# lh3/miniwfa

Measured on AMD Instinct MI355X. Metric: aligned Gbp/s (q+t), higher is better.
Workload: dtype int16x2 packed, range-guarded (bit-exact to the reference's int32); 1 GPU; 1024 pairs/GPU x 10000 bp, 0.05 divergence, score-only mwf_wfa_exact, default penalties (BASELINE configs[2]); pairs_this_gpu=1024, pairs_total=1024, target_len=10000, bases_this_gpu=20479492, grid=512, block=512

## Files before the change

miniwfa_amd/build.py:

```python
from __future__ import annotations

import os
import subprocess
import sys

HERE = os.path.dirname(os.path.abspath(__file__))
ROOT = os.path.dirname(HERE)
CSRC = os.path.join(HERE, "csrc")
LIB = os.path.join(CSRC, "libmwf_hip.so")
SOURCES = ["mwf_band2.hip", "mwf_band2_e3.hip", "mwf_band2_e4.hip", "mwf_band2_bi.hip", "mwf_band2_bi_deep.hip", "mwf_kernels.hip", "mwf_lane.hip", "mwf_mid.hip", "mwf_sys.hip", "mwf_sys_deep.hip", "mwf_cigar_ops.hip", "mwf_engine.cpp", "mwf_memory.cpp", "mwf_plan.cpp", "mwf_chain.cpp", "mwf_async.cpp", "kalloc.cpp", "mwf_dbg.cpp"]
HEADERS = [os.path.join(CSRC, "mwf_internal.h"), os.path.join(CSRC, "mwf_device.h"), os.path.join(CSRC, "mwf_sys_pass.h"), os.path.join(CSRC, "mwf_engine.h"), os.path.join(ROOT, "include", "miniwfa.h"), os.path.join(ROOT, "include", "kalloc.h")]
SOURCE_DEPS = {"mwf_band2_e3.hip": ["mwf_band2.hip"], "mwf_band2_e4.hip": ["mwf_band2.hip"], "mwf_band2_bi.hip": ["mwf_band2.hip"], "mwf_band2_bi_deep.hip": ["mwf_band2.hip"]}


def hipcc() -> str:
    for cand in (os.environ.get("HIPCC"), "/opt/rocm/bin/hipcc", "hipcc"):
        if cand and (os.path.isabs(cand) and os.path.exists(cand) or not os.path.isabs(cand)):
            return cand
    return "hipcc"


def stale() -> bool:
    if not os.path.exists(LIB):
        return True
    t = os.path.getmtime(LIB)
    deps = [os.path.join(CSRC, s) for s in SOURCES if os.path.exists(os.path.join(CSRC, s))] + HEADERS + [os.path.abspath(__file__)]
    return any(os.path.getmtime(d) > t for d in deps)


def build(force: bool = False, verbose: bool = False) -> str:
    if not force and not stale():
        return LIB
    from concurrent.futures import ThreadPoolExecutor
    objdir = os.path.join(CSRC, "build")
    os.makedirs(objdir, exist_ok=True)
    flags = ["--offload-arch=gfx950", "-O3", "-std=c++17", "-fPIC", "-Wall", "-Wno-unused-function", "-I", os.path.join(ROOT, "include"), "-I", CSRC]
    hdr_time = max(os.path.getmtime(h) for h in HEADERS + [os.path.abspath(__file__)])
    jobs, objs = [], []
    for name in SOURCES:
        src = os.path.join(CSRC, name)
        if not os.path.exists(src):
            continue
        obj = os.path.join(objdir, name + ".o")
        objs.append(obj)
        src_time = max(os.path.getmtime(os.path.join(CSRC, d)) for d in [name, *SOURCE_DEPS.get(name, [])])
        if force or not os.path.exists(obj) or os.path.getmtime(obj) < max(src_time, hdr_time):
            jobs.append([hipcc(), *flags, "-c", src, "-o", obj])

    def run(cmd):
        if verbose:
            print(" ".join(cmd))
        return cmd, subprocess.run(cmd, capture_output=True, text=True)

    with ThreadPoolExecutor(max(1, min(6, len(jobs)))) as ex:
        for cmd, r in ex.map(run, jobs):
            if r.returncode != 0:
                sys.stderr.write(r.stdout + r.stderr)
                raise RuntimeError("hipcc failed: " + " ".join(cmd))
            if verbose and r.stderr.strip():
                sys.stderr.write(r.stderr)
    cmd, r = run([hipcc(), "--offload-arch=gfx950", "-fPIC", "-shared", *objs, "-o", LIB + ".tmp", "-lpthread"])
    if r.returncode != 0:
        sys.stderr.write(r.stdout + r.stderr)
        raise RuntimeError("hipcc failed linking libmwf_hip.so")
    os.replace(LIB + ".tmp", LIB)
    return LIB


KERNEL_FILES = {"wfa_band2_kernel": "mwf_band2.hip", "wfa_sys_kernel": "mwf_sys.hip", "wfa_sys_seg_kernel": "mwf_sys.hip", "wfa_batch_kernel": "mwf_kernels.hip",
                "wfa_lane_kernel": "mwf_lane.hip", "wfa_mid_kernel": "mwf_mid.hip"}
KERNEL_HEADERS = {"mwf_sys.hip": ["mwf_sys_pass.h", "mwf_sys_deep.hip"], "mwf_band2.hip": ["mwf_band2_e3.hip", "mwf_band2_e4.hip", "mwf_band2_bi.hip", "mwf_band2_bi_deep.hip"]}


def kernel_fingerprint(symbol: str) -> str | None:
    import hashlib
    name = symbol.split("<")[0].strip()
    f = KERNEL_FILES.get(name)
    if f is None:
        return None
    h = hashlib.sha256()
    for p in [os.path.join(CSRC, x) for x in [f, *KERNEL_HEADERS.get(f, []), "mwf_device.h", "mwf_internal.h"]]:
        try:
            h.update(open(p, "rb").read())
        except OSError:
            return None
    return h.hexdigest()[:16]


CLI = os.path.join(ROOT, "tools", "test-mwf")


def build_cli(force: bool = False) -> str:
    src = os.path.join(ROOT, "tools", "test-mwf.cpp")
    if not force and os.path.exists(CLI) and os.path.getmtime(CLI) >= max(os.path.getmtime(src), os.path.getmtime(LIB)):
        return CLI
    zl = ["-DMWF_HAVE_ZLIB", "-lz"] if os.path.exists("/usr/include/zlib.h") else []
    cmd = ["g++", "-O2", "-std=c++17", "-Wall", "-I", os.path.join(ROOT, "include"), src, "-o", CLI,
           "-L", CSRC, "-lmwf_hip", "-Wl,-rpath," + CSRC] + zl
    r = subprocess.run(cmd, capture_output=True, text=True)
    if r.returncode != 0:
        sys.stderr.write(r.stdout + r.stderr)
        raise RuntimeError("g++ failed building tools/test-mwf")
    return CLI


if __name__ == "__main__":
    print(build(force="--force" in sys.argv, verbose=True))
    print(build_cli(force="--force" in sys.argv))
```

miniwfa_amd/csrc/mwf_band2.hip:

```cpp
#include <cstddef>
#include <cstdio>
#include <cstdlib>
#include <type_traits>
#include "mwf_device.h"

namespace mwf {

using namespace dev;

namespace {

extern __shared__ __attribute__((aligned(16))) uint8_t lds2[];

constexpr int kWideT = 512, kWideK = 3;
constexpr int kWaves768 = 1;
constexpr int kSpanK = 5;
constexpr int kW4K = 5;
constexpr int kSpanT = 1024;
constexpr bool is_span(int T, int K) { return T == kSpanT && K == kSpanK; }
constexpr int kWideWaves = 4;
constexpr int kChunk = 256;
constexpr int kFoldMaxLag = 8;
constexpr int32_t kDeadPair = (int32_t)0x80008000u;

__device__ __forceinline__ int32_t from_left(int32_t v, int32_t fill) { return __builtin_amdgcn_update_dpp(fill, v, 0x138, 0xf, 0xf, false); }
__device__ __forceinline__ int32_t from_right(int32_t v, int32_t fill) { return __builtin_amdgcn_update_dpp(fill, v, 0x130, 0xf, 0xf, false); }
__device__ __forceinline__ int32_t lo16(int32_t v) { return (int32_t)(int16_t)(v & 0xffff); }
__device__ __forceinline__ int32_t hi16(int32_t v) { return v >> 16; }
__device__ __forceinline__ int32_t pack2(int32_t a, int32_t b)
{
	typedef short short2_t __attribute__((ext_vector_type(2)));
	const short2_t v = __builtin_amdgcn_cvt_pk_i16(a, b);
	return __builtin_bit_cast(int32_t, v);
}
__device__ __forceinline__ int32_t both16(int32_t v) { return (int32_t)(((uint32_t)v << 16) | ((uint32_t)v & 0xffffu)); }

__device__ __forceinline__ uint32_t seq4(int32_t off)
{
	const uint32_t *p = (const uint32_t*)(lds2 + (off & ~3));
	return __builtin_amdgcn_alignbyte(p[1], p[0], (uint32_t)off);
}

__device__ __forceinline__ int32_t lead_eq(uint32_t x)
{
	int32_t fb;
	asm("v_ffbl_b32 %0, %1" : "=v"(fb) : "v"(x));
	return (int32_t)((uint32_t)fb >> 3);
}

template <bool WANT_TB>
__device__ __forceinline__ Cell cell16(int32_t hx, int32_t o1m, int32_t g1m, int32_t o2m, int32_t g2m,
                                       int32_t o1p, int32_t g1p, int32_t o2p, int32_t g2p)
{
	if (!WANT_TB) return wf_cell<false>(hx, o1m, g1m, o2m, g2m, o1p, g1p, o2p, g2p);
	Cell c;
	c.e1 = max(o1m, g1m);
	c.e2 = max(o2m, g2m);
	c.f1 = max(o1p, g1p) + 1;
	c.f2 = max(o2p, g2p) + 1;
	const int32_t e = max(c.e1, c.e2), f = max(c.f1, c.f2), g = max(e, f), m = hx + 1;
	c.h = max(m, g);
	const uint32_t z = c.h == m ? 0u : c.h == c.e1 ? 1u : c.h == c.e2 ? 3u : c.h == c.f1 ? 2u : 4u;
	c.tb = z | ((uint32_t)(c.e1 != o1m) << 3) | ((uint32_t)(c.f1 != o1p + 1) << 4) | ((uint32_t)(c.e2 != o2m) << 5) | ((uint32_t)(c.f2 != o2p + 1) << 6);
	(void)e, (void)f, (void)g;
	return c;
}

struct Probe8 { uint32_t t0, t1, t2, q0, q1, q2; };
__device__ __forceinline__ void probe8_issue(Probe8 &p, int32_t j, int32_t aq)
{
	const uint32_t *pt = (const uint32_t*)(lds2 + (j & ~3)), *pq = (const uint32_t*)(lds2 + (aq & ~3));
	p.t0 = pt[0], p.t1 = pt[1], p.t2 = pt[2], p.q0 = pq[0], p.q1 = pq[1], p.q2 = pq[2];
}
__device__ __forceinline__ int32_t probe8_count(const Probe8 &p, int32_t j, int32_t aq)
{
	const uint32_t x0 = __builtin_amdgcn_alignbyte(p.t1, p.t0, (uint32_t)j) ^ __builtin_amdgcn_alignbyte(p.q1, p.q0, (uint32_t)aq);
	const uint32_t x1 = __builtin_amdgcn_alignbyte(p.t2, p.t1, (uint32_t)j) ^ __builtin_amdgcn_alignbyte(p.q2, p.q1, (uint32_t)aq);
	return min(min(lead_eq(x0), lead_eq(x1) + 4), 9);
}

__device__ __forceinline__ uint32_t seq16(int32_t base, int32_t j)
{
	const uint32_t *p = (const uint32_t*)(lds2 + base + ((j >> 4) << 2));
	return __builtin_amdgcn_alignbit(p[1], p[0], (uint32_t)j << 1);
}
__device__ __forceinline__ int32_t lead_eq2(uint32_t x)
{
	int32_t fb;
	asm("v_ffbl_b32 %0, %1" : "=v"(fb) : "v"(x));
	return (int32_t)((uint32_t)fb >> 1);
}
struct Probe16 { uint32_t t0, t1, q0, q1; };
__device__ __forceinline__ void probe16_issue(Probe16 &p, int32_t qbase, int32_t j, int32_t iq)
{
	const uint32_t *pt = (const uint32_t*)(lds2 + ((j >> 4) << 2)), *pq = (const uint32_t*)(lds2 + qbase + ((iq >> 4) << 2));
	p.t0 = pt[0], p.t1 = pt[1], p.q0 = pq[0], p.q1 = pq[1];
}
__device__ __forceinline__ int32_t probe16_count(const Probe16 &p, int32_t j, int32_t iq)
{
	return min(lead_eq2(__builtin_amdgcn_alignbit(p.t1, p.t0, (uint32_t)j << 1) ^ __builtin_amdgcn_alignbit(p.q1, p.q0, (uint32_t)iq << 1)), 17);
}
__device__ __forceinline__ int32_t run_wave16(int32_t qbase, int32_t j, int32_t iq, int32_t room, int32_t n0)
{
	const int32_t lane = threadIdx.x & 63;
	int32_t n = n0;
	while (n < room) {
		const int32_t off = n + 16 * lane;
		int32_t m = 0;
		if (off < room) m = min(min(lead_eq2(seq16(0, j + off) ^ seq16(qbase, iq + off)), 16), room - off);
		const unsigned long long stop = __ballot(m < 16);
		if (stop == 0) { n += 1024; continue; }
		const int32_t first = (int32_t)__builtin_ctzll(stop);
		n += 16 * first + __builtin_amdgcn_readlane(m, first);
		break;
	}
	return min(n, room);
}
template <int T>
__device__ __forceinline__ uint32_t pack2bit(const uint8_t *src, int32_t len, int32_t base)
{
	uint32_t bad = 0;
	const int32_t n_dw = (len >> 4) + 2;
	for (int32_t w = threadIdx.x; w < n_dw; w += T) {
		uint32_t out = 0;
		const int32_t b0 = w << 4;
		if (b0 + 16 <= len) {
			uint32_t q[4];
			__builtin_memcpy(q, src + b0, 16);
#pragma unroll
			for (int k = 0; k < 4; ++k) {
				const uint32_t x = q[k], code = (x >> 1) & 0x03030303u;
				const uint32_t lo1 = code & 0x01010101u, hi1 = (code >> 1) & 0x01010101u;
				const uint32_t expect = 0x41414141u + (lo1 & ~hi1) * 0x02u + (hi1 & ~lo1) * 0x13u + (hi1 & lo1) * 0x06u;
				bad |= x ^ expect;
				out |= ((code | code >> 6 | code >> 12 | code >> 18) & 0xffu) << (8 * k);
			}
		} else {
#pragma unroll 1
			for (int32_t k = 0; k < 16 && b0 + k < len; ++k) {
				const uint32_t x = src[b0 + k], code = (x >> 1) & 3u;
				bad |= x ^ ((0x47544341u >> (8 * code)) & 0xffu);
				out |= code << (2 * k);
			}
		}
		*(uint32_t*)(lds2 + base + 4 * w) = out;
	}
	return bad;
}

__device__ __forceinline__ uint32_t inm_bit(int32_t d, int32_t k, int32_t tl, int32_t ql)
{
	return (uint32_t)((uint32_t)(k + 1) < (uint32_t)(tl + 1)) & (uint32_t)((uint32_t)(d + k + 1) < (uint32_t)(ql + 1));
}

__device__ __forceinline__ unsigned long long lane_mask(int32_t base, int32_t k, int32_t a, int32_t b)
{
	int32_t lmin = a - base - k, lmax = b - base - k;
	if (lmax < 0) return 0ull;
	lmin = lmin <= 0 ? 0 : (lmin + 3) >> 2;
	lmax = min(lmax >> 2, 63);
	if (lmin > lmax) return 0ull;
	return (~0ull >> (63 - lmax)) & (~0ull << lmin);
}

__device__ __forceinline__ int32_t run_wave2(int32_t j, int32_t aq, int32_t room, int32_t n0)
{
	const int32_t lane = threadIdx.x & 63;
	int32_t n = n0;
	while (n < room) {
		const int32_t off = n + 4 * lane;
		int32_t m = 0;
		if (off < room) {
			const uint32_t x = seq4(j + off) ^ seq4(aq + off);
			m = min(min(lead_eq(x), 4), room - off);
		}
		const unsigned long long stop = __ballot(m < 4);
		if (stop == 0) { n += 256; continue; }
		const int32_t first = (int32_t)__builtin_ctzll(stop);
		n += 4 * first + __builtin_amdgcn_readlane(m, first);
		break;
	}
	return min(n, room);
}

constexpr int32_t kBiasOver = 1500, kBiasMargin = 600;
__device__ __forceinline__ int32_t wide_bias(int32_t tl) { return max(tl + kBiasOver - 32767, 0); }

template <int D, int NWK>
struct alignas(16) Band2Lds {
	Shared sh;
	int32_t edge[D][NWK + 2][4];
	int32_t dump[64 * 2 + (2 * NWK + 4) * 4];
};

typedef short s16x2 __attribute__((ext_vector_type(2)));
typedef unsigned short u16x2 __attribute__((ext_vector_type(2)));
#define MWF_BC(T, v) __builtin_bit_cast(T, v)
__device__ __forceinline__ int32_t pk_max(int32_t a, int32_t b) { return MWF_BC(int32_t, __builtin_elementwise_max(MWF_BC(s16x2, a), MWF_BC(s16x2, b))); }
__device__ __forceinline__ int32_t pk_add(int32_t a, int32_t b) { return MWF_BC(int32_t, (s16x2)(MWF_BC(s16x2, a) + MWF_BC(s16x2, b))); }
__device__ __forceinline__ int32_t pk_sub(int32_t a, int32_t b) { return MWF_BC(int32_t, (s16x2)(MWF_BC(s16x2, a) - MWF_BC(s16x2, b))); }
__device__ __forceinline__ int32_t pk_minu(int32_t a, int32_t b) { return MWF_BC(int32_t, __builtin_elementwise_min(MWF_BC(u16x2, a), MWF_BC(u16x2, b))); }
__device__ __forceinline__ int32_t pk_subsat(int32_t a, int32_t b) { return MWF_BC(int32_t, __builtin_elementwise_sub_sat(MWF_BC(u16x2, a), MWF_BC(u16x2, b))); }
__device__ __forceinline__ int32_t pk_nonzero_mask(int32_t x)
{
	int32_t m;
	asm("v_pk_min_u16 %0, %1, 1 op_sel_hi:[1,0]\n\tv_pk_sub_i16 %0, 0, %0 op_sel_hi:[0,1]" : "=&v"(m) : "v"(x));
	return m;
}
__device__ __forceinline__ int32_t pk_ne1(int32_t a, int32_t b)
{
	int32_t m;
	asm("v_xor_b32 %0, %1, %2\n\tv_pk_min_u16 %0, %0, 1 op_sel_hi:[1,0]" : "=&v"(m) : "v"(a), "v"(b));
	return m;
}
__device__ __forceinline__ int32_t pk_mad(int32_t a, int32_t b, int32_t c)
{
	int32_t m;
	asm("v_pk_mad_u16 %0, %1, %2, %3" : "=v"(m) : "v"(a), "v"(b), "v"(c));
	return m;
}
__device__ __forceinline__ int32_t bfi(int32_t mask, int32_t a, int32_t b) { return (a & mask) | (b & ~mask); }
__device__ __forceinline__ int32_t half_of(int32_t v, int hi) { return hi ? v >> 16 : (int32_t)(int16_t)(v & 0xffff); }
__device__ __forceinline__ int32_t pair_of(int32_t lo, int32_t hi) { return (int32_t)(((uint32_t)hi << 16) | ((uint32_t)lo & 0xffffu)); }

__device__ __forceinline__ int32_t left_of_A(int32_t B, int32_t fill) { return __builtin_amdgcn_alignbit(B, from_left(B, fill), 16); }
__device__ __forceinline__ int32_t right_of_B(int32_t A, int32_t fill) { return __builtin_amdgcn_alignbit(from_right(A, fill), A, 16); }

template <int T, int K, int E1, int E2, bool TB, bool S2, bool BI4, bool FOLD, typename ArgsT>
__device__ PassResult band2_pass(const ArgsT &A, const PairMem &M, Shared &sh, const int32_t edge_base, const int32_t qoff, bool trace_band)
{
	constexpr int NW = T / 64, NWK = NW * K, D = (E1 > E2 ? E1 : E2) + 1;
	constexpr bool BI = is_span(T, K) || BI4;
	constexpr int FULL = S2 ? 16 : 8;
	constexpr int kAgeOut = FOLD ? kFoldMaxLag : D;
	constexpr int kAge = (NWK + 2) * 16;
	static_assert(D >= 2 && D <= 5, "edge-table ages");
	const int32_t tl = M.tl, ql = M.ql, cmax = tl + ql + 1;
	const int32_t tid = threadIdx.x, lane = tid & 63, wave = uni(tid >> 6);
	const int32_t W = A.W, nH = A.pen.nH, lagx = A.pen.x, lag1 = A.pen.oe1, lag2 = A.pen.oe2;
	const int32_t B = BI ? wide_bias(tl) : 0;
	const int32_t ONEB = BI ? both16(1 + B) : 0x00010001;
	char *const Hb = (char*)M.H;
	const uint32_t RS = (uint32_t)W << 1;
	const int32_t min_lag = min(lagx, min(lag1, lag2));
	const bool relaxed_stores = min_lag >= 3;
	PassResult R;
	R.status = ST_OK, R.s = 0, R.info = 0, R.n_snap = 0, R.cells = 0;

	static_assert(E1 >= 1 && E1 <= 4 && (E2 == 1 || E2 == 2), "history depth");
	int32_t e1h[E1][K][2], f1h[E1][K][2], e2h[E2][K][2], f2h[E2][K][2];
#pragma unroll
	for (int k = 0; k < K; ++k)
#pragma unroll
		for (int i = 0; i < 2; ++i) {
#pragma unroll
			for (int a = 0; a < E1; ++a) e1h[a][k][i] = f1h[a][k][i] = kDeadPair;
#pragma unroll
			for (int a = 0; a < E2; ++a) e2h[a][k][i] = f2h[a][k][i] = kDeadPair;
		}
	const int32_t RA = pair_of(4 * lane, 4 * lane + 2);
	const uint32_t lane8 = ((uint32_t)lane << 3) + 8u;
	const int32_t nd = lane == 0 ? -4 : 8;
	const int32_t T0 = both16(cmax), TLp = both16(tl), TL1 = both16(tl + 1);
	const int32_t ebase = edge_base + wave * 16, dump_base = edge_base + D * kAge + NW * 16;
	const int32_t dump_lane = dump_base + lane * 8;
	int32_t epos[D];
#pragma unroll
	for (int a = 0; a < D; ++a) epos[a] = a * kAge;

	{
		const int32_t reach = nH + 1 + 8, g_a = max(tl + 1 - reach, 0) >> 8, n_g = ((tl + 1 + reach) >> 8) - g_a + 1, per_row = n_g * 64;
		for (int32_t q = tid; q < nH * per_row; q += T) {
			const int32_t row = q / per_row, rem = q - row * per_row;
			*(int2*)(Hb + (size_t)((uint32_t)row * RS + (uint32_t)(g_a * 512 + rem * 8 + 8))) = make_int2(kDeadPair, kDeadPair);
		}
	}
	for (int32_t j = tid; j < D * (NWK + 2) * 4; j += T) *(int32_t*)(lds2 + edge_base + 4 * j) = kDeadPair;
	if (tid == 0) {
		for (int32_t j = 0; j < nH; ++j) sh.rng_lo[j] = 1, sh.rng_hi[j] = 0;
		for (int32_t j = 0; j < 12; ++j) (&sh.flags[0][0])[j] = 0;
		sh.rng_lo[0] = sh.rng_hi[0] = tl + 1;
		sh.word[3] = -1;
	}
	__syncthreads();
	if (tid < 64) {
		const int32_t k0 = (S2 ? run_wave16(qoff, 0, 0, min(tl, ql), 0) : run_wave2(0, qoff, min(tl, ql), 0)) - 1;
		if (tid == 0) {
			const int32_t c = tl + 1, e = c & 3;
			*(int16_t*)(Hb + 8 + (size_t)(uint32_t)(((c & ~3) + ((e & 1) << 1) + (e >> 1)) << 1)) = (int16_t)(k0 - B);
			sh.word[1] = k0;
		}
	}
	__syncthreads();
	{
		const int32_t k0 = uni(sh.word[1]);
		if (k0 == tl - 1 && k0 == ql - 1) return R;
	}

	int32_t s = 0, wf_lo = tl + 1, wf_hi = tl + 1;
	int32_t curH = 0, par = 0;
	const uint32_t ring_bytes = (uint32_t)nH * RS;
	uint32_t bn = (uint32_t)(1 % nH) * RS, bx = (uint32_t)((nH - lagx + 1) % nH) * RS, b1 = (uint32_t)((nH - lag1 + 1) % nH) * RS, b2 = (uint32_t)((nH - lag2 + 1) % nH) * RS;
	struct Rows { int2 HX, O1, O2; int32_t N1, N2; } pre;
	pre.HX = pre.O1 = pre.O2 = make_int2(0, 0), pre.N1 = pre.N2 = 0;
	auto load_rows = [&](Rows &r, const char *rx, const char *r1, const char *r2, uint32_t off) {
		const uint32_t noff = off + (uint32_t)nd;
		r.HX = *(const int2*)(rx + off), r.O2 = *(const int2*)(r2 + off);
		r.N2 = *(const int32_t*)(r2 + noff);
		if (!FOLD) r.O1 = *(const int2*)(r1 + off), r.N1 = *(const int32_t*)(r1 + noff);
	};
	int64_t cells = 0, tb_used = 0;
	int32_t est_window = 0;
	const int64_t iter_limit = A.max_iter > 0 ? A.max_iter : INT64_MAX;
	const int32_t s_limit = A.max_s > 0 ? A.max_s : INT32_MAX;
	const int64_t rows_slot = TB ? A.rows_slot : 0, tb_slot_bytes = TB ? A.tb_slot_bytes : 0;

	int32_t gl = (wf_lo > 1 ? wf_lo - 1 : 1) >> 8, gk[K];
	auto remap = [&](int32_t g_lo) {
		const int32_t base = g_lo - g_lo % NWK;
#pragma unroll
		for (int k = 0; k < K; ++k) {
			int32_t g = base + wave + NW * k;
			if (g < g_lo) g += NWK;
			gk[k] = g;
		}
	};
	remap(gl);
	int32_t idle[K];
#pragma unroll
	for (int k = 0; k < K; ++k) idle[k] = kAgeOut;
	int32_t up_wait = 0, up_min = 0;
	int32_t ekey = 0;
	constexpr bool kEpoch = !is_span(T, K) && T != 64;
	uint32_t est = 0;
	static_assert(kEpoch || ((NW & (NW - 1)) == 0 && !(T == 512 && K == 4)), "the full header of the gated geometries is written for a power-of-two wave count and no three-slot note");
	static_assert(K <= 6, "slot classes of the window epoch: four bits per slot below bit 24");

	auto step = [&]() __attribute__((always_inline)) -> bool {
		constexpr int P1 = E1 - 1, P2 = E2 - 1;
#ifdef MWF_B2_TIMING
		const uint64_t tm0 = __builtin_readcyclecounter();
#endif
		const int32_t lo = wf_lo > 1 ? wf_lo - 1 : 1;
		const int32_t hi = wf_hi < cmax ? wf_hi + 1 : cmax;
		const int32_t lo_p = lo, hi_p = hi;
		const int32_t s_new = s + 1;
		const int32_t newH = curH + 1 == nH ? 0 : curH + 1;
		const int32_t npar = par + 1 == 3 ? 0 : par + 1;
		const int32_t origin = lo & ~3;
		const int32_t row_bytes = (hi | 3) - origin + 1;
		if (TB) {
			if (s_new - 1 >= rows_slot) { R.status = ST_ROWS_OVERFLOW; return true; }
			if (tb_used + row_bytes > tb_slot_bytes) { R.status = ST_TB_OVERFLOW; return true; }
		}
		const int32_t gl_next = (lo > 1 ? lo - 1 : 1) >> 8;
		const int32_t ga = lo >> 8, gb = hi >> 8;
		const int32_t key = gl_next | gb << 15 | 1 << 29 | (ga - gl_next) << 30;
		const bool fast = kEpoch && key == ekey;
		uint32_t st = est;
		bool act[K];
		if (!kEpoch) {
			if (gb - min(ga, gl + 1) + 3 > NWK - 1)
				if (((hi < cmax ? hi + 1 : cmax) >> 8) - min(gl_next, gl) + 1 > NWK - 1) { R.status = ST_BAND_OVERFLOW; return true; }
			if (BI && cmax - lo > 65535) { R.status = ST_BAND_OVERFLOW; return true; }
		} else if (!fast) {
			bool hold = true;
			if (gb - min(ga, gl + 1) + 3 > NWK - 1) {
				if (((hi < cmax ? hi + 1 : cmax) >> 8) - min(gl_next, gl) + 1 > NWK - 1) { R.status = ST_BAND_OVERFLOW; return true; }
				hold = false;
			}
			if (T == 512 && K == 4 && R.n_snap == 0 && gb - ga + 3 > 23) {
				if (((hi < cmax ? hi + 1 : cmax) >> 8) - gl_next + 1 > 23) R.n_snap = 1;
				hold = false;
			}
			if (BI) {
				if (cmax - lo > 65535) { R.status = ST_BAND_OVERFLOW; return true; }
				if (cmax - (ga << 8) > 65535) hold = false;
			}
			const int32_t gspan = gb - ga;
			int n_busy = 0;
			st = 0;
#pragma unroll
			for (int k = 0; k < K; ++k) {
				if ((uint32_t)(gk[k] - ga) <= (uint32_t)gspan) {
					idle[k] = 0;
					st |= (1u | (gk[k] == ga ? 2u : 0u) | (gk[k] == gb ? 4u : 0u)) << (4 * k);
					if (k < 2 || k == K - 1) ++n_busy;
				} else if (idle[k] < kAgeOut) {
					++idle[k];
					st |= 9u << (4 * k);
					hold = false;
				}
			}
			if ((NW & (NW - 1)) == 0) {
				const int32_t pos = (wave - ga) & (NW - 1);
				const int32_t left = gspan + 1 - pos + ((pos == 0 || ((gb - wave) & (NW - 1)) == 0) ? NW : 0);
				if (left > 2 * NW) __builtin_amdgcn_s_setprio(3);
				else if (left > NW) __builtin_amdgcn_s_setprio(2);
				else if (left > 0) __builtin_amdgcn_s_setprio(1);
				else __builtin_amdgcn_s_setprio(0);
			} else {
				if (n_busy >= 3) __builtin_amdgcn_s_setprio(3);
				else if (n_busy == 2) __builtin_amdgcn_s_setprio(2);
				else if (n_busy == 1) __builtin_amdgcn_s_setprio(1);
				else __builtin_amdgcn_s_setprio(0);
			}
			if (ga >= 1 && wave == (ga - 1) % NW) st |= 1u << 24;
			if (wave == (gb + 1) % NW) st |= 1u << 25;
			est = st, ekey = kEpoch && hold ? ~key : -1;
		}
		const char *const rowx = Hb + bx, *const row1 = Hb + b1, *const row2 = Hb + b2;
		char *const rown = Hb + bn;
		const bool track_good = (((256 - (s_new & 255)) & 255) < nH);
		const int32_t rE1 = ebase + epos[E1 - 1], rE2 = ebase + epos[E2 - 1];
		const int32_t wE = lane == 63 ? ebase + epos[D - 1] : dump_lane, wF = lane == 0 ? ebase + epos[D - 1] : dump_lane;
		auto put_edge = [&](int k, int32_t e1b, int32_t e2b, int32_t f1a, int32_t f2a) {
			*(int2*)(lds2 + wE + (k * NW + 1) * 16) = make_int2(e1b, e2b);
			*(int2*)(lds2 + wF + (k * NW + 1) * 16 + 8) = make_int2(f1a, f2a);
			if (k == K - 1 && wave == NW - 1) *(int2*)(lds2 + wE - (NW - 1) * 16) = make_int2(e1b, e2b);
			if (k == 0 && wave == 0) *(int2*)(lds2 + wF + (NWK + 1) * 16 + 8) = make_int2(f1a, f2a);
		};
		const bool forecast = NWK < 24 ? (s_new == 64 || s_new == 256 || s_new == 1024) : NWK >= 64 ? (s_new == 1024 || s_new == 4096) : false;
		int32_t far = kDeadPair;
		const int32_t cfin = ql + 1;

		if (wave == 0) {
			sh.rng_lo[newH] = lo, sh.rng_hi[newH] = hi;
			sh.flags[npar + 1 == 3 ? 0 : npar + 1][0] = 0;
			if (TB) M.row_off[s_new - 1] = tb_used, M.row_lo[s_new - 1] = origin;
#ifndef MWF_B2_TIMING
			if (trace_band && s_new - 1 < fresh(A).dbg_cap) M.dbg[2 * (s_new - 1)] = lo, M.dbg[2 * (s_new - 1) + 1] = hi;
#endif
		}

		if (!kEpoch) {
#pragma unroll
			for (int k = 0; k < K; ++k) act[k] = (uint32_t)(gk[k] - ga) <= (uint32_t)(gb - ga);
			const int32_t pos = (wave - ga) & (NW - 1);
			const int32_t left = gb - ga + 1 - pos + ((pos == 0 || ((gb - wave) & (NW - 1)) == 0) ? NW : 0);
			if (left > 2 * NW) __builtin_amdgcn_s_setprio(3);
			else if (left > NW) __builtin_amdgcn_s_setprio(2);
			else if (left > 0) __builtin_amdgcn_s_setprio(1);
			else __builtin_amdgcn_s_setprio(0);
		}
#ifdef MWF_B2_TIMING
		int n_act = 0;
#pragma unroll
		for (int k = 0; k < K; ++k) n_act += (kEpoch ? (st >> (4 * k) & 9u) == 1u : act[k]) ? 1 : 0;
#endif

#ifdef MWF_B2_TIMING
		const uint64_t tm1 = __builtin_readcyclecounter();
#endif
		int n_stores = 0;
		if (kEpoch ? (st & (1u << 24)) != 0 : (ga >= 1 && wave == (ga - 1) % NW)) *(int2*)(rown + ((uint32_t)((ga - 1) << 9) + lane8)) = make_int2(kDeadPair, kDeadPair);
		if (kEpoch ? (st & (1u << 25)) != 0 : wave == (gb + 1) % NW) *(int2*)(rown + ((uint32_t)((gb + 1) << 9) + lane8)) = make_int2(kDeadPair, kDeadPair);
#if MWF_B2_TIMING == 2
		bool chunk_timed = false;
		uint32_t ct[4] = {0, 0, 0, 0};
#endif
#pragma unroll
		for (int k = 0; k < K; ++k) {
			const uint32_t cls = st >> (4 * k);
			if (kEpoch) {
				if (!(cls & 1u)) continue;
			} else if (!act[k]) {
				if (idle[k] >= kAgeOut) continue;
				++idle[k];
			} else idle[k] = 0;
			const bool edgy = (cls & 0xeu) != 0;
			int32_t lo = uni(lo_p), hi = uni(hi_p);
			asm volatile("" : "+s"(lo), "+s"(hi));
			const int32_t g = gk[k], cb = g * kChunk, c0 = cb + 4 * lane;
#if MWF_B2_TIMING == 2
			uint64_t tc0 = 0, tc1 = 0, tc2 = 0, tc3 = 0, tc4 = 0;
			const bool timed = !chunk_timed;
			if (timed) asm volatile("s_memtime %0\n\ts_waitcnt lgkmcnt(0)" : "=s"(tc0) :: "memory");
#endif
			const uint32_t off = (uint32_t)(cb << 1) + lane8;
			load_rows(pre, rowx, row1, row2, off);
			const int2 HX = pre.HX, O1 = pre.O1, O2 = pre.O2;
			const int32_t N1 = pre.N1, N2 = pre.N2;
			const int32_t xE1 = *(const int32_t*)(lds2 + rE1 + k * NW * 16), xE2 = *(const int32_t*)(lds2 + rE2 + k * NW * 16 + 4);
			const int32_t xF1 = *(const int32_t*)(lds2 + rE1 + (k * NW + 2) * 16 + 8), xF2 = *(const int32_t*)(lds2 + rE2 + (k * NW + 2) * 16 + 12);
			const bool inside = (kEpoch && !edgy) || (cb >= lo && cb + kChunk - 1 <= hi);

			const int32_t E1a = e1h[P1][k][0], E1b = e1h[P1][k][1], F1a = f1h[P1][k][0], F1b = f1h[P1][k][1];
			const int32_t E2a = e2h[P2][k][0], E2b = e2h[P2][k][1], F2a = f2h[P2][k][0], F2b = f2h[P2][k][1];
			const int32_t o1mA = FOLD ? 0 : left_of_A(O1.y, N1), o2mA = left_of_A(O2.y, N2), g1mA = left_of_A(E1b, xE1), g2mA = left_of_A(E2b, xE2);
			const int32_t o1pB = FOLD ? 0 : right_of_B(O1.x, N1), o2pB = right_of_B(O2.x, N2), g1pB = right_of_B(F1a, xF1), g2pB = right_of_B(F2a, xF2);
			const int32_t ONE = 0x00010001;
			int32_t ne1A = FOLD ? g1mA : pk_max(o1mA, g1mA), ne2A = pk_max(o2mA, g2mA);
			int32_t ne1B = FOLD ? E1a : pk_max(O1.x, E1a), ne2B = pk_max(O2.x, E2a);
			const int32_t pf1A = FOLD ? F1b : pk_max(O1.y, F1b), pf2A = pk_max(O2.y, F2b);
			const int32_t pf1B = FOLD ? g1pB : pk_max(o1pB, g1pB), pf2B = pk_max(o2pB, g2pB);
			int32_t nf1A = pk_add(pf1A, ONE), nf2A = pk_add(pf2A, ONE), nf1B = pk_add(pf1B, ONE), nf2B = pk_add(pf2B, ONE);
			const int32_t mA = pk_add(HX.x, ONE), mB = pk_add(HX.y, ONE);
			int32_t hA = pk_max(pk_max(mA, pk_max(ne1A, ne2A)), pk_max(nf1A, nf2A));
			int32_t hB = pk_max(pk_max(mB, pk_max(ne1B, ne2B)), pk_max(nf1B, nf2B));
#if MWF_B2_TIMING == 2
			if (timed) asm volatile("s_memtime %0\n\ts_waitcnt lgkmcnt(0)" : "=s"(tc1) : "v"(hA), "v"(hB) : "memory");
#endif
			uint32_t tbw = 0;
			if (TB) {
				const int32_t TWO = 0x00020002, NEG1 = (int32_t)0xffffffffu, EIGHT = 0x00080008, C16 = 0x00100010, C32 = 0x00200020, C64 = 0x00400040;
				int32_t zA = pk_mad(pk_ne1(hA, nf1A), TWO, NEG1), zB = pk_mad(pk_ne1(hB, nf1B), TWO, NEG1);
				zA = pk_mad(pk_ne1(hA, ne2A), zA, TWO), zB = pk_mad(pk_ne1(hB, ne2B), zB, TWO);
				zA = pk_mad(pk_ne1(hA, ne1A), zA, ONE), zB = pk_mad(pk_ne1(hB, ne1B), zB, ONE);
				zA = pk_mad(pk_ne1(hA, mA), zA, 0), zB = pk_mad(pk_ne1(hB, mB), zB, 0);
				if (!FOLD) {
					zA = pk_mad(pk_ne1(ne1A, o1mA), EIGHT, zA), zB = pk_mad(pk_ne1(ne1B, O1.x), EIGHT, zB);
					zA = pk_mad(pk_ne1(pf1A, O1.y), C16, zA), zB = pk_mad(pk_ne1(pf1B, o1pB), C16, zB);
				}
				zA = pk_mad(pk_ne1(ne2A, o2mA), C32, zA), zB = pk_mad(pk_ne1(ne2B, O2.x), C32, zB);
				zA = pk_mad(pk_ne1(pf2A, O2.y), C64, zA), zB = pk_mad(pk_ne1(pf2B, o2pB), C64, zB);
				tbw = (uint32_t)zA | ((uint32_t)zB << 8);
			}
			const int32_t cbp = both16(cb);
			const int32_t xA = pk_sub(pk_sub(T0, cbp), RA);
			const int32_t rjA = pk_minu(xA, TLp), rjB = pk_minu(pk_sub(xA, ONE), TLp);
			const int32_t dA = pk_sub(pk_add(RA, cbp), TL1), dB = pk_add(dA, ONE);
			const bool on_lo = kEpoch ? (cls & 2u) != 0 : g == ga, on_hi = kEpoch ? (cls & 4u) != 0 : g == gb;
			const bool special = is_span(T, K) || (BI4 && !TB) || (kEpoch ? edgy : !inside || on_lo || on_hi) || track_good;
			int32_t outA = 0, outB = 0;
			uint32_t bits = 0, gbits = 0;
			if (special) {
			if (!inside) {
				const int32_t lo_r = both16(min(max(lo - cb, 0), 256)), hi_r1 = both16(min(max(hi - cb + 1, 0), 256));
				const int32_t RB = pk_add(RA, 0x00010001), RB1 = pk_add(RA, 0x00020002);
				outA = pk_nonzero_mask(pk_subsat(lo_r, RA) | pk_subsat(RB, hi_r1));
				outB = pk_nonzero_mask(pk_subsat(lo_r, RB) | pk_subsat(RB1, hi_r1));
				hA = bfi(outA, kDeadPair, hA), hB = bfi(outB, kDeadPair, hB);
				ne1A = bfi(outA, kDeadPair, ne1A), ne1B = bfi(outB, kDeadPair, ne1B);
				ne2A = bfi(outA, kDeadPair, ne2A), ne2B = bfi(outB, kDeadPair, ne2B);
				nf1A = bfi(outA, kDeadPair, nf1A), nf1B = bfi(outB, kDeadPair, nf1B);
				nf2A = bfi(outA, kDeadPair, nf2A), nf2B = bfi(outB, kDeadPair, nf2B);
			}
			if (on_lo || on_hi) {
				if (on_lo) {
					const int32_t rel = lo - cb;
					const int32_t v = half_of(__builtin_amdgcn_readlane((rel & 1) ? hB : hA, rel >> 2), (rel >> 1) & 1);
					bits |= v >= -1 - B ? 1u : 0u;
				}
				if (on_hi) {
					const int32_t rel = hi - cb;
					const int32_t v = half_of(__builtin_amdgcn_readlane((rel & 1) ? hB : hA, rel >> 2), (rel >> 1) & 1);
					bits |= v >= -1 - B ? 2u : 0u;
				}
			}
			if (track_good) {
				auto bad = [&](int32_t v, int32_t rj) { return pk_subsat(pk_add(v, ONEB), rj); };
				const int32_t bA = pk_minu(pk_minu(bad(hA, rjA), pk_minu(bad(ne1A, rjA), bad(nf1A, rjA))), pk_minu(bad(ne2A, rjA), bad(nf2A, rjA))) | outA;
				const int32_t bB = pk_minu(pk_minu(bad(hB, rjB), pk_minu(bad(ne1B, rjB), bad(nf1B, rjB))), pk_minu(bad(ne2B, rjB), bad(nf2B, rjB))) | outB;
				gbits = (uint32_t)((bA & 0xffff) == 0) | (uint32_t)((bB & 0xffff) == 0) << 1 | (uint32_t)(((uint32_t)bA >> 16) == 0) << 2 | (uint32_t)(((uint32_t)bB >> 16) == 0) << 3;
				if (BI && (s_new & 255) == 0) {
					const int32_t width = both16(kBiasMargin), from = both16(-1 - B - kBiasMargin), top = both16(32768 - kBiasMargin);
					auto stray = [&](int32_t v, int32_t lo_end) { return pk_subsat(width, pk_sub(v, lo_end)); };
					const int32_t any = stray(hA, from) | stray(hB, from) | stray(ne1A, from) | stray(ne1B, from) | stray(ne2A, from) | stray(ne2B, from) |
					                    stray(nf1A, from) | stray(nf1B, from) | stray(nf2A, from) | stray(nf2B, from) | stray(hA, top) | stray(hB, top);
					if (__ballot(any != 0)) bits |= 0x80u;
				}
			}
			}
			if (FOLD) {
				ne1A = pk_max(ne1A, HX.x), ne1B = pk_max(ne1B, HX.y), nf1A = pk_max(nf1A, HX.x), nf1B = pk_max(nf1B, HX.y);
				if (TB) {
					const int32_t EIGHT = 0x00080008, C16 = 0x00100010;
					const int32_t fA = pk_mad(pk_ne1(ne1A, HX.x), EIGHT, pk_mad(pk_ne1(nf1A, HX.x), C16, 0));
					const int32_t fB = pk_mad(pk_ne1(ne1B, HX.y), EIGHT, pk_mad(pk_ne1(nf1B, HX.y), C16, 0));
					tbw |= (uint32_t)fA | ((uint32_t)fB << 8);
				}
			}
			e1h[P1][k][0] = ne1A, e1h[P1][k][1] = ne1B, f1h[P1][k][0] = nf1A, f1h[P1][k][1] = nf1B;
			e2h[P2][k][0] = ne2A, e2h[P2][k][1] = ne2B, f2h[P2][k][0] = nf2A, f2h[P2][k][1] = nf2B;
#pragma unroll
			for (int i = 0; i < 2; ++i) {
#pragma unroll
				for (int a = E1 - 1; a > 0; --a) {
					asm volatile("v_swap_b32 %0, %1" : "+v"(e1h[a - 1][k][i]), "+v"(e1h[a][k][i]));
					asm volatile("v_swap_b32 %0, %1" : "+v"(f1h[a - 1][k][i]), "+v"(f1h[a][k][i]));
				}
#pragma unroll
				for (int a = E2 - 1; a > 0; --a) {
					asm volatile("v_swap_b32 %0, %1" : "+v"(e2h[a - 1][k][i]), "+v"(e2h[a][k][i]));
					asm volatile("v_swap_b32 %0, %1" : "+v"(f2h[a - 1][k][i]), "+v"(f2h[a][k][i]));
				}
			}
			put_edge(k, ne1B, ne2B, nf1A, nf2A);

#if MWF_B2_TIMING == 2
			if (timed) asm volatile("s_memtime %0\n\ts_waitcnt lgkmcnt(0)" : "=s"(tc2) : "v"(hA), "v"(hB), "v"(rjA), "v"(dA) : "memory");
#endif
			const int32_t jA = pk_minu(pk_add(hA, ONEB), rjA), jB = pk_minu(pk_add(hB, ONEB), rjB);
			const int32_t iqA = pk_add(jA, dA), iqB = pk_add(jB, dB);
			int32_t cnt[4];
			if (S2) {
				uint64_t tw[4], qw[4];
#pragma unroll
				for (int u = 0; u < 4; ++u) {
					const uint32_t J = (uint32_t)((u & 1) ? jB : jA), Q = (uint32_t)((u & 1) ? iqB : iqA);
					const uint32_t ta = (u & 2) ? (J >> 18) & 0x3ffcu : (J >> 2) & 0x3ffcu;
					const uint32_t qa = ((u & 2) ? (Q >> 20) : ((Q >> 4) & 0xfffu)) * 4u + (uint32_t)qoff;
					asm volatile("ds_read2_b32 %0, %1 offset1:1" : "=v"(tw[u]) : "v"(ta));
					asm volatile("ds_read2_b32 %0, %1 offset1:1" : "=v"(qw[u]) : "v"(qa));
				}
				asm volatile("s_waitcnt lgkmcnt(0)" : "+v"(tw[0]), "+v"(tw[1]), "+v"(tw[2]), "+v"(tw[3]), "+v"(qw[0]), "+v"(qw[1]), "+v"(qw[2]), "+v"(qw[3]));
#pragma unroll
				for (int u = 0; u < 4; ++u) {
					const uint32_t J = (uint32_t)((u & 1) ? jB : jA), Q = (uint32_t)((u & 1) ? iqB : iqA);
					const uint32_t tsh = (u & 2) ? (BI ? (J >> 15) & 30u : J >> 15) : J << 1, qsh = (u & 2) ? (Q >> 15) & 30u : Q << 1;
					cnt[u] = lead_eq2(__builtin_amdgcn_alignbit((uint32_t)(tw[u] >> 32), (uint32_t)tw[u], tsh) ^ __builtin_amdgcn_alignbit((uint32_t)(qw[u] >> 32), (uint32_t)qw[u], qsh));
				}
			} else {
				constexpr int PF = (K >= 3 && T >= 512) ? 1 : 2;
#pragma unroll
				for (int h2 = 0; h2 < 4 / PF; ++h2) {
					Probe8 pr[PF];
					int32_t jj[PF], aq[PF];
#pragma unroll
					for (int v = 0; v < PF; ++v) {
						const int u = PF * h2 + v;
						jj[v] = (int32_t)((uint32_t)((u & 1) ? jB : jA) >> ((u & 2) ? 16 : 0) & 0xffffu);
						aq[v] = (int32_t)((uint32_t)((u & 1) ? iqB : iqA) >> ((u & 2) ? 16 : 0) & 0xffffu) + qoff;
						probe8_issue(pr[v], jj[v], aq[v]);
					}
#pragma unroll
					for (int v = 0; v < PF; ++v) cnt[PF * h2 + v] = probe8_count(pr[v], jj[v], aq[v]);
				}
			}
			typedef unsigned short us2_t __attribute__((ext_vector_type(2)));
			const int32_t cA = MWF_BC(int32_t, (us2_t)__builtin_amdgcn_cvt_pk_u16((uint32_t)cnt[0], (uint32_t)cnt[2]));
			const int32_t cB = MWF_BC(int32_t, (us2_t)__builtin_amdgcn_cvt_pk_u16((uint32_t)cnt[1], (uint32_t)cnt[3]));
#if MWF_B2_TIMING == 2
			if (timed) asm volatile("s_memtime %0\n\ts_waitcnt lgkmcnt(0)" : "=s"(tc3) : "v"(cA), "v"(cB) : "memory");
#endif
			const int32_t FULLp = both16(FULL);
			const int32_t m9A = pk_minu(cA, pk_sub(rjA, jA)), m9B = pk_minu(cB, pk_sub(rjB, jB));
			int32_t nmA = pk_minu(m9A, FULLp), nmB = pk_minu(m9B, FULLp);
			const int32_t pendp = pk_subsat(m9A, FULLp) | pk_subsat(m9B, FULLp);
			if (__ballot(pendp != 0)) {
				int32_t hv[4] = {half_of(hA, 0) + B, half_of(hB, 0) + B, half_of(hA, 1) + B, half_of(hB, 1) + B};
				int32_t nmat[4] = {(int32_t)((uint32_t)nmA & 0xffffu), (int32_t)((uint32_t)nmB & 0xffffu), (int32_t)((uint32_t)nmA >> 16), (int32_t)((uint32_t)nmB >> 16)};
				const uint32_t pend = (uint32_t)(((uint32_t)m9A & 0xffffu) > (uint32_t)FULL) | (uint32_t)(((uint32_t)m9B & 0xffffu) > (uint32_t)FULL) << 1 |
				                      (uint32_t)(((uint32_t)m9A >> 16) > (uint32_t)FULL) << 2 | (uint32_t)(((uint32_t)m9B >> 16) > (uint32_t)FULL) << 3;
				uint32_t open = 0;
#pragma unroll
				for (int i = 0; i < 4; ++i) {
					if (__ballot((pend >> i) & 1u) == 0) continue;
					if ((pend >> i) & 1u) {
						int32_t n = FULL;
						const int32_t j = hv[i] + 1, q = c0 + i - 1 - tl + j, rm = min(tl - j, ql - q), aqq = qoff + q;
						for (int trip = 0; n < rm; ++trip) {
							if (trip == 4) { open |= 1u << i; break; }
							if (S2) {
								const int32_t m = min(lead_eq2(seq16(0, j + n) ^ seq16(qoff, q + n)), 16);
								n += m;
								if (m < 16) break;
							} else {
								const uint32_t xa = seq4(j + n) ^ seq4(aqq + n), xb = seq4(j + n + 4) ^ seq4(aqq + n + 4);
								if (xa | xb) { n += xa ? min(lead_eq(xa), 4) : 4 + min(lead_eq(xb), 4); break; }
								n += 8;
							}
						}
						nmat[i] = min(n, rm);
					}
				}
				for (unsigned long long owners = __ballot(open != 0); owners; owners &= owners - 1) {
					const int32_t src = (int32_t)__builtin_ctzll(owners);
					const int32_t c0s = cb + 4 * src;
					const uint32_t ob = (uint32_t)__builtin_amdgcn_readlane((int32_t)open, src);
#pragma unroll
					for (int i = 0; i < 4; ++i) {
						if (!((ob >> i) & 1u)) continue;
						const int32_t hh = __builtin_amdgcn_readlane(hv[i], src);
						const int32_t j = hh + 1, q = c0s + i - 1 - tl + j, rm = min(tl - j, ql - q);
						const int32_t n = S2 ? run_wave16(qoff, j, q, rm, 80) : run_wave2(j, qoff + q, rm, 40);
						nmat[i] = lane == src ? n : nmat[i];
					}
				}
				nmA = pair_of(nmat[0], nmat[2]), nmB = pair_of(nmat[1], nmat[3]);
			}
			const int32_t hxA = pk_add(hA, nmA), hxB = pk_add(hB, nmB);
			if (forecast) far = pk_max(far, pk_max(hxA, hxB));
			unsigned long long fm = 0;
			int32_t done_info = 0;
			if ((uint32_t)(cfin - cb) < (uint32_t)kChunk && cfin >= lo && cfin <= hi) {
				const int32_t rel = cfin - cb, hi_half = (rel >> 1) & 1;
				const int32_t hv = half_of((rel & 1) ? hxB : hxA, hi_half) + B, nm = (int32_t)((uint32_t)((rel & 1) ? nmB : nmA) >> (hi_half ? 16 : 0) & 0xffffu);
				const uint32_t f = (uint32_t)(lane == (rel >> 2)) & (uint32_t)(hv == tl - 1) & inm_bit(ql - tl, hv - nm, tl, ql);
				done_info = (f && nm == 0) ? (int32_t)((tbw >> (8 * (rel & 3))) & 7u) : 0;
				fm = __ballot(f != 0);
			}
			*(int2*)(rown + off) = make_int2(hxA, hxB);
			++n_stores;
#if MWF_B2_TIMING == 2
			if (timed) {
				asm volatile("s_memtime %0\n\ts_waitcnt lgkmcnt(0)" : "=s"(tc4) : "v"(hxA), "v"(hxB) : "memory");
				chunk_timed = true;
				ct[0] = (uint32_t)min(tc1 - tc0, (uint64_t)4095), ct[1] = (uint32_t)min(tc2 - tc1, (uint64_t)4095);
				ct[2] = (uint32_t)min(tc3 - tc2, (uint64_t)4095), ct[3] = (uint32_t)min(tc4 - tc3, (uint64_t)4095);
			}
#endif
			if (TB && c0 >= origin && c0 <= hi) *(uint32_t*)(M.tb + tb_used - origin + c0) = tbw;
			if (track_good) {
				unsigned long long *gword = M.good + (int64_t)newH * fresh(A).GW + g * 4;
#pragma unroll
				for (int i = 0; i < 4; ++i) {
					const unsigned long long m = __ballot((gbits >> i) & 1u);
					if (lane == 0) gword[i] = m;
				}
			}
			if (fm) bits |= 4u | (uint32_t)__builtin_amdgcn_readlane(done_info, (int32_t)__builtin_ctzll(fm)) << 4;
			if (bits && lane == 0) atomicOr((unsigned int*)&sh.flags[npar][0], bits);
		}

		if (forecast) {
			const int32_t m = wave_max(max(lo16(far), hi16(far))) + B;
			if (lane == 0 && m >= 0) atomicMax(&sh.word[3], m);
		}
#ifdef MWF_B2_TIMING
		const uint64_t tm2 = __builtin_readcyclecounter();
#endif
		bn = bn + RS == ring_bytes ? 0u : bn + RS, bx = bx + RS == ring_bytes ? 0u : bx + RS;
		b1 = b1 + RS == ring_bytes ? 0u : b1 + RS, b2 = b2 + RS == ring_bytes ? 0u : b2 + RS;
		const bool young_store = relaxed_stores && n_stores > 0 && !TB && !track_good;
		if (young_store) asm volatile("s_waitcnt vmcnt(1) lgkmcnt(0)" ::: "memory");
		else asm volatile("s_waitcnt vmcnt(0) lgkmcnt(0)" ::: "memory");
#ifdef MWF_B2_TIMING
		const uint64_t tm3 = __builtin_readcyclecounter();
#endif
		__builtin_amdgcn_s_barrier();
		asm volatile("" ::: "memory");

		const uint32_t fl = (uint32_t)uni(sh.flags[npar][0]);
#ifdef MWF_B2_TIMING
		if (trace_band && tid == (fresh(A).max_iter < 0 ? (int32_t)-fresh(A).max_iter : 0) && s_new - 1 < fresh(A).dbg_cap) {
			const uint64_t tm4 = __builtin_readcyclecounter();
#if MWF_B2_TIMING == 2
			M.dbg[2 * (s_new - 1)] = (int32_t)(ct[0] | ct[1] << 12 | (uint32_t)n_act << 28);
			M.dbg[2 * (s_new - 1) + 1] = (int32_t)(ct[2] | ct[3] << 12);
			(void)tm4;
#else
			M.dbg[2 * (s_new - 1)] = (int32_t)(min((uint32_t)(tm1 - tm0), 65535u) | min((uint32_t)(tm2 - tm1), 65535u) << 16);
			M.dbg[2 * (s_new - 1) + 1] = (int32_t)(min((uint32_t)(tm3 - tm2), 4095u) | min((uint32_t)(tm4 - tm3), 65535u) << 12 | (uint32_t)n_act << 28);
#endif
		}
#endif
		if (fl & 1u) wf_lo = lo;
		if (fl & 2u) wf_hi = hi;
		const int32_t done = (int32_t)((fl >> 2) & 1u), payload = (int32_t)((fl >> 4) & 7u);
		if (BI && (fl & 0x80u)) { R.status = ST_BAND_OVERFLOW; return true; }
		s = s_new, curH = newH, par = npar;
		{
			const int32_t oldest = epos[D - 1];
#pragma unroll
			for (int a = D - 1; a > 0; --a) epos[a] = epos[a - 1];
			epos[0] = oldest;
		}
		if (!kEpoch || ekey < 0) {
			if (gl_next < gl) gl = gl_next, remap(gl), up_wait = 0, ekey = 0;
			else if (gl_next > gl) {
				up_min = up_wait == 0 ? gl_next : min(up_min, gl_next);
				if (++up_wait > kAgeOut) gl = up_min, remap(gl), up_wait = 0;
				ekey = 0;
			} else up_wait = 0, ekey = ~ekey;
		}
		if (TB) tb_used += row_bytes;
		if ((s & 0xff) == 0) {
			if (tid == 0) sh.red[0] = 0x7fffffff, sh.red[1] = -1;
			__syncthreads();
			const int32_t gfirst = wf_lo >> 8, n_words = ((wf_hi >> 8) - gfirst + 1) * 4, GWc = fresh(A).GW;
			for (int32_t q = tid; q < n_words; q += T) {
				const int32_t gg = gfirst + (q >> 2), kq = q & 3, base = gg * kChunk;
				unsigned long long m = 0;
				for (int32_t j = 0; j < nH; ++j)
					if (sh.rng_lo[j] <= sh.rng_hi[j] && sh.rng_lo[j] <= base + kChunk - 1 && sh.rng_hi[j] >= base) m |= M.good[(int64_t)j * GWc + gg * 4 + kq];
				m &= lane_mask(base, kq, wf_lo, wf_hi);
				if (m) {
					atomicMin(&sh.red[0], base + 4 * (int32_t)__builtin_ctzll(m) + kq);
					atomicMax(&sh.red[1], base + 4 * (63 - (int32_t)__builtin_clzll(m)) + kq);
				}
			}
			__syncthreads();
			const int32_t glo = uni(sh.red[0]), ghi = uni(sh.red[1]);
			if (ghi < 0) { R.status = ST_INTERNAL; return true; }
			wf_lo = glo, wf_hi = ghi;
		}
		cells += hi - lo + 1;
		if (cells > iter_limit || s > s_limit) {
			R.status = ST_STOPPED;
			return true;
		}
		if (done) {
			R.info = payload;
			return true;
		}
		if (forecast) {
			est_window = window_forecast(s, uni(sh.word[3]), tl, ql, (NWK - 1) * kChunk - 64, NWK >= 24 && NWK < 64);
			if (est_window) { R.status = ST_BAND_OVERFLOW; return true; }
		}
		return false;
	};
	for (;;)
		if (step()) break;
	asm volatile("s_waitcnt vmcnt(0)" ::: "memory");
	R.s = s, R.cells = est_window ? -(int64_t)est_window : cells;
	return R;
}

constexpr int band2_waves(int T, int K, bool TB)
{
	return is_span(T, K) ? (T == 1024 ? 4 : 3) : T == 1024 ? 4 : T == kWideT ? kWideWaves : T <= 512 ? ((TB && T < 512) ? 3 : 4) : kWaves768;
}
template <int T, int K, int E1, int E2, bool TB, bool S2, bool BI4 = false, bool FOLD = false>
__global__ __launch_bounds__(T, band2_waves(T, K, TB)) void wfa_band2_kernel(const BatchArgs)
{
	constexpr int NWK = (T / 64) * K, D = (E1 > E2 ? E1 : E2) + 1;
	KArgs &A0 = kernel_args();
	if ((uint32_t)(uintptr_t)lds2 != 0u) __builtin_trap();
	typedef Band2Lds<D, NWK> LdsT;
	const int32_t lds_seq = A0.band_lds_seq;
	LdsT *const L = (LdsT*)(lds2 + lds_seq);
	Shared &sh = L->sh;
	const int32_t edge_base = lds_seq + (int32_t)offsetof(LdsT, edge);
	CigLocal cig_loc;
	cig_loc.base = 0, cig_loc.left = 0;
	for (int32_t round = 0;; ++round) {
		KArgs &A = fresh(A0);
		if (threadIdx.x == 0) sh.item = A.queue ? (int32_t)atomicAdd(A.queue, 1) : (round == 0 ? (int32_t)blockIdx.x : A.n_pairs), sh.word[2] = 0;
		__syncthreads();
		const int32_t item = uni(sh.item);
		__syncthreads();
		if (item >= A.n_pairs) break;
		const int32_t pair = A.order ? A.order[item] : item;
		PairMem M;
		pair_mem(A, (int32_t)blockIdx.x, pair, M);
		const int32_t qoff = S2 ? ((M.tl >> 4) + 2) * 4 : ((M.tl + 3) & ~3) + 8;
		PassResult R;
		R.status = ST_OK, R.s = 0, R.info = 0, R.n_snap = 0, R.cells = 0;
		if (S2) {
			uint32_t bad = pack2bit<T>(M.ts, M.tl, 0);
			bad |= pack2bit<T>(M.qs, M.ql, qoff);
			if (bad) sh.word[2] = 1;
			__syncthreads();
			if (uni(sh.word[2])) R.status = ST_ALPHABET;
		} else {
			for (int32_t j = threadIdx.x; j < M.tl; j += T) lds2[j] = M.ts[j];
			for (int32_t j = threadIdx.x; j < M.ql; j += T) lds2[qoff + j] = M.qs[j];
			__syncthreads();
		}
		const bool trace = A.dbg && pair == A.debug_pair;
		if (R.status == ST_OK) R = band2_pass<T, K, E1, E2, TB, S2, BI4, FOLD>(A, M, sh, edge_base, qoff, trace);
		if (T == 512 && K == 4 && R.n_snap && threadIdx.x == 0 && fresh(A0).report_wide) atomicOr((unsigned int*)(fresh(A0).cig_head + 1), 1u);
		R.n_snap = 0;
		if (S2) M.t2 = lds2, M.q2 = lds2 + qoff;
		if (TB && FOLD) M.tb_fwd = 1;
		finish_pair(fresh(A0), M, (int32_t)blockIdx.x, pair, R, R.status, 0, T <= 256 ? &cig_loc : nullptr);
	}
}

template <int T, int K, int E1, int E2>
constexpr int lds_tail() { return (int)sizeof(Band2Lds<(E1 > E2 ? E1 : E2) + 1, (T / 64) * K>); }

template <int T, int K, int E1, int E2, bool TB, bool S2, bool BI4 = false, bool FOLD = false>
void launch_variant(const BatchArgs &a, int grid, int lds, hipStream_t st)
{
	if constexpr (!FOLD && T >= 512 && S2 && E1 == 2) {
		if (a.band_fold && a.pen.oe1 - a.pen.x == E1 && a.pen.oe1 < kFoldMaxLag) return launch_variant<T, K, E1, E2, TB, S2, BI4, true>(a, grid, lds, st);
	}
	if (lds > 48 * 1024) {
		(void)hipFuncSetAttribute(reinterpret_cast<const void*>(&wfa_band2_kernel<T, K, E1, E2, TB, S2, BI4, FOLD>), hipFuncAttributeMaxDynamicSharedMemorySize, lds);
		(void)hipGetLastError();
	}
	if (getenv("MWF_DEBUG"))
		fprintf(stderr, "[libmwf_hip] band2 launch: T %d K %d E1 %d E2 %d TB %d S2 %d BI4 %d FOLD %d, %d pairs, grid %d\n", T, K, E1, E2, (int)TB, (int)S2, (int)BI4, (int)FOLD, (int)a.n_pairs, grid);
	hipLaunchKernelGGL((wfa_band2_kernel<T, K, E1, E2, TB, S2, BI4, FOLD>), dim3(grid), dim3(T), lds, st, a);
}

template <int T, int K, int E1, int E2, bool BI4 = false>
int launch_one(const BatchArgs &a0, int grid, int lds_seq, bool seq2, hipStream_t st)
{
	BatchArgs a = a0;
	a.band_lds_seq = lds_seq;
	const int lds = lds_seq + lds_tail<T, K, E1, E2>();
	if constexpr (is_span(T, K) || (T == 512 && K >= 4)) {
		if (!seq2) return -1;
		if (a.want_cigar) launch_variant<T, K, E1, E2, true, true, BI4>(a, grid, lds, st);
		else launch_variant<T, K, E1, E2, false, true, BI4>(a, grid, lds, st);
	} else if constexpr (T == 768) {
		if (seq2) return -1;
		if (a.want_cigar) launch_variant<T, K, E1, E2, true, false>(a, grid, lds, st);
		else launch_variant<T, K, E1, E2, false, false>(a, grid, lds, st);
	} else {
		if (!seq2) return -1;
		if (a.want_cigar) launch_variant<T, K, E1, E2, true, true>(a, grid, lds, st);
		else launch_variant<T, K, E1, E2, false, true>(a, grid, lds, st);
	}
	return hipGetLastError() == hipSuccess ? 0 : -2;
}

template <int T, int K, int E1, int E2, bool BI4 = false>
int occ_one(int lds_seq, bool seq2, bool tb)
{
	const int lds = lds_seq + lds_tail<T, K, E1, E2>();
	int n = 0;
	hipError_t e;
	if constexpr (is_span(T, K) || (T == 512 && K >= 4)) {
		if (!seq2) return 0;
		e = tb ? hipOccupancyMaxActiveBlocksPerMultiprocessor(&n, wfa_band2_kernel<T, K, E1, E2, true, true, BI4>, T, lds)
		       : hipOccupancyMaxActiveBlocksPerMultiprocessor(&n, wfa_band2_kernel<T, K, E1, E2, false, true, BI4>, T, lds);
	} else if constexpr (T == 768) {
		if (seq2) return 0;
		e = tb ? hipOccupancyMaxActiveBlocksPerMultiprocessor(&n, wfa_band2_kernel<T, K, E1, E2, true, false>, T, lds)
		       : hipOccupancyMaxActiveBlocksPerMultiprocessor(&n, wfa_band2_kernel<T, K, E1, E2, false, false>, T, lds);
	} else {
		if (!seq2) return 0;
		e = tb ? hipOccupancyMaxActiveBlocksPerMultiprocessor(&n, wfa_band2_kernel<T, K, E1, E2, true, true>, T, lds)
		       : hipOccupancyMaxActiveBlocksPerMultiprocessor(&n, wfa_band2_kernel<T, K, E1, E2, false, true>, T, lds);
	}
	return e == hipSuccess ? n : 0;
}

}

#define MWF_BAND2_CAT_(a, b) a##b
#define MWF_BAND2_CAT(a, b) MWF_BAND2_CAT_(a, b)
int launch_band2_e3(const BatchArgs &a, int grid, const BandGeom &g, void *stream);
int launch_band2_e4(const BatchArgs &a, int grid, const BandGeom &g, void *stream);
int band2_occupancy_e3(const Penalty &p, const BandGeom &g, bool cigar);
int band2_occupancy_e4(const Penalty &p, const BandGeom &g, bool cigar);
int launch_band2_bi1(const BatchArgs &a, int grid, const BandGeom &g, void *stream);
int launch_band2_bi2(const BatchArgs &a, int grid, const BandGeom &g, void *stream);
int band2_occupancy_bi1(const Penalty &p, const BandGeom &g, bool cigar);
int band2_occupancy_bi2(const Penalty &p, const BandGeom &g, bool cigar);

#if !defined(MWF_BAND2_DEEP) && !defined(MWF_BAND2_BIASED)
bool band2_supported(const Penalty &p)
{
	const bool deep = (p.e1 == 3 && (p.e2 == 1 || p.e2 == 2)) || (p.e1 == 4 && p.e2 == 1);
	return ((p.e1 == 2 && p.e2 == 1) || (p.e1 == 2 && p.e2 == 2) || (p.e1 == 1 && p.e2 == 1) || deep) && p.nH <= kMaxRing;
}
#endif

#if defined(MWF_BAND_DEV) || defined(MWF_BAND2_BIASED)
#define MWF_BAND2_REST(FN, ...)
#else
#define MWF_BAND2_REST(FN, ...)                                                     \
	if (g.block == 256) MWF_BAND2_PEN(FN, 256, 3, __VA_ARGS__)                      \
	if (g.block == 128) MWF_BAND2_PEN(FN, 128, 3, __VA_ARGS__)                      \
	if (g.block == 64) MWF_BAND2_PEN(FN, 64, 3, __VA_ARGS__)
#endif
#if defined(MWF_BAND2_BIASED)
#define MWF_BAND2_PEN(FN, T, K, ...) {}
#elif defined(MWF_BAND2_DEEP) && MWF_BAND2_DEEP == 3
#define MWF_BAND2_PEN(FN, T, K, ...)                                                \
	{                                                                               \
		if (a_e1 == 3 && a_e2 == 1) return FN<T, K, 3, 1>(__VA_ARGS__);             \
		if (a_e1 == 3 && a_e2 == 2) return FN<T, K, 3, 2>(__VA_ARGS__);             \
	}
#elif defined(MWF_BAND2_DEEP)
#define MWF_BAND2_PEN(FN, T, K, ...)                                                \
	{                                                                               \
		if (a_e1 == MWF_BAND2_DEEP && a_e2 == 1) return FN<T, K, MWF_BAND2_DEEP, 1>(__VA_ARGS__); \
	}
#elif defined(MWF_BAND_DEV)
#define MWF_BAND2_PEN(FN, T, K, ...) { if (a_e1 == 2 && a_e2 == 1) return FN<T, K, 2, 1>(__VA_ARGS__); }
#else
#define MWF_BAND2_PEN(FN, T, K, ...)                                                \
	{                                                                               \
		if (a_e1 == 2 && a_e2 == 1) return FN<T, K, 2, 1>(__VA_ARGS__);             \
		if (a_e1 == 2 && a_e2 == 2) return FN<T, K, 2, 2>(__VA_ARGS__);             \
		if (a_e1 == 1 && a_e2 == 1) return FN<T, K, 1, 1>(__VA_ARGS__);             \
	}
#endif
#if defined(MWF_BAND2_BIASED) && MWF_BAND2_BIASED == 1
#define MWF_BAND2_PEN4(FN, K, ...)                                                  \
	{                                                                               \
		if (a_e1 == 2 && a_e2 == 2) return FN<512, K, 2, 2, true>(__VA_ARGS__);     \
		if (a_e1 == 1 && a_e2 == 1) return FN<512, K, 1, 1, true>(__VA_ARGS__);     \
	}
#elif defined(MWF_BAND2_BIASED)
#define MWF_BAND2_PEN4(FN, K, ...)                                                  \
	{                                                                               \
		if (a_e1 == 3 && a_e2 == 1) return FN<512, K, 3, 1, true>(__VA_ARGS__);     \
		if (a_e1 == 3 && a_e2 == 2) return FN<512, K, 3, 2, true>(__VA_ARGS__);     \
		if (a_e1 == 4 && a_e2 == 1) return FN<512, K, 4, 1, true>(__VA_ARGS__);     \
	}
#endif
#if defined(MWF_BAND2_BIASED)
#define MWF_BAND2_PEN4B(FN, ...) MWF_BAND2_PEN4(FN, kW4K, __VA_ARGS__)
#define MWF_BAND2_PEN4C(FN, ...) MWF_BAND2_PEN4(FN, kW4K + 1, __VA_ARGS__)
#elif defined(MWF_BAND2_DEEP)
#define MWF_BAND2_PEN4B(FN, ...) {}
#define MWF_BAND2_PEN4C(FN, ...) {}
#else
#define MWF_BAND2_PEN4B(FN, ...)                                                    \
	{                                                                               \
		if (a_e1 == 2 && a_e2 == 1) return FN<512, kW4K, 2, 1, true>(__VA_ARGS__);     \
	}
#define MWF_BAND2_PEN4C(FN, ...)                                                    \
	{                                                                               \
		if (a_e1 == 2 && a_e2 == 1) return FN<512, kW4K + 1, 2, 1, true>(__VA_ARGS__); \
	}
#endif
#define MWF_BAND2_DISPATCH(FN, ...)                                                 \
	do {                                                                            \
		if (g.block == 512 && g.span > 8 * kW4K * 256 && g.packed == 2) MWF_BAND2_PEN4C(FN, __VA_ARGS__)  \
		if (g.block == 512 && g.span > 512 / 64 * 3 * 256 && g.packed == 2) MWF_BAND2_PEN4B(FN, __VA_ARGS__)  \
		if (g.block == 512 && g.span > 512 / 64 * 3 * 256) MWF_BAND2_PEN(FN, 512, 4, __VA_ARGS__)  \
		if (g.block == 512) MWF_BAND2_PEN(FN, kWideT, kWideK, __VA_ARGS__) \
		if (g.block == 768) MWF_BAND2_PEN(FN, 768, 2, __VA_ARGS__)                  \
		if (g.block == 1024) MWF_BAND2_PEN(FN, kSpanT, kSpanK, __VA_ARGS__) \
		MWF_BAND2_REST(FN, __VA_ARGS__)                                             \
	} while (0)

#if defined(MWF_BAND2_BIASED)
int MWF_BAND2_CAT(launch_band2_bi, MWF_BAND2_BIASED)(const BatchArgs &a, int grid, const BandGeom &g, void *stream)
{
	const int a_e1 = a.pen.e1, a_e2 = a.pen.e2;
	if (g.packed != 2) return -1;
	MWF_BAND2_DISPATCH(launch_one, a, grid, g.lds_bytes, g.seq2 != 0, (hipStream_t)stream);
	return -1;
}

int MWF_BAND2_CAT(band2_occupancy_bi, MWF_BAND2_BIASED)(const Penalty &p, const BandGeom &g, bool cigar)
{
	const int a_e1 = p.e1, a_e2 = p.e2;
	if (g.packed != 2) return 0;
	MWF_BAND2_DISPATCH(occ_one, g.lds_bytes, g.seq2 != 0, cigar);
	return 0;
}
#elif defined(MWF_BAND2_DEEP)
int MWF_BAND2_CAT(launch_band2_e, MWF_BAND2_DEEP)(const BatchArgs &a, int grid, const BandGeom &g, void *stream)
{
	const int a_e1 = a.pen.e1, a_e2 = a.pen.e2;
	if (g.packed == 2) return -1;
	MWF_BAND2_DISPATCH(launch_one, a, grid, g.lds_bytes, g.seq2 != 0, (hipStream_t)stream);
	return -1;
}

int MWF_BAND2_CAT(band2_occupancy_e, MWF_BAND2_DEEP)(const Penalty &p, const BandGeom &g, bool cigar)
{
	const int a_e1 = p.e1, a_e2 = p.e2;
	if (g.packed == 2) return 0;
	MWF_BAND2_DISPATCH(occ_one, g.lds_bytes, g.seq2 != 0, cigar);
	return 0;
}
#else
int launch_band2(const BatchArgs &a, int grid, const BandGeom &g, void *stream)
{
	const int a_e1 = a.pen.e1, a_e2 = a.pen.e2;
	if (g.packed == 2 && !(a_e1 == 2 && a_e2 == 1)) return a_e1 <= 2 ? launch_band2_bi1(a, grid, g, stream) : launch_band2_bi2(a, grid, g, stream);
	if (a_e1 == 3) return launch_band2_e3(a, grid, g, stream);
	if (a_e1 == 4) return launch_band2_e4(a, grid, g, stream);
	MWF_BAND2_DISPATCH(launch_one, a, grid, g.lds_bytes, g.seq2 != 0, (hipStream_t)stream);
	return -1;
}

int band2_span_chunks() { return kSpanT / 64 * kSpanK; }
int band2_biased512_chunks() { return 8 * kW4K; }
bool band2_biased512_supported(const Penalty &p)
{
	return (p.e1 == 2 && (p.e2 == 1 || p.e2 == 2)) || (p.e1 == 1 && p.e2 == 1) || (p.e1 == 3 && (p.e2 == 1 || p.e2 == 2)) || (p.e1 == 4 && p.e2 == 1);
}

int band2_kernel_occupancy(const Penalty &p, const BandGeom &g, bool cigar)
{
	const int a_e1 = p.e1, a_e2 = p.e2;
	if (g.packed == 2 && !(a_e1 == 2 && a_e2 == 1)) return a_e1 <= 2 ? band2_occupancy_bi1(p, g, cigar) : band2_occupancy_bi2(p, g, cigar);
	if (a_e1 == 3) return band2_occupancy_e3(p, g, cigar);
	if (a_e1 == 4) return band2_occupancy_e4(p, g, cigar);
	MWF_BAND2_DISPATCH(occ_one, g.lds_bytes, g.seq2 != 0, cigar);
	return 0;
}
#endif

}
```

miniwfa_amd/csrc/mwf_engine.cpp:

```cpp
#include "mwf_engine.h"

extern "C" {


int mwf_gpu_device_count(void)
{
	int n = 0;
	if (hipGetDeviceCount(&n) != hipSuccess) { (void)hipGetLastError(); return 0; }
	return n;
}

mwf_gpu_t *mwf_gpu_create(int device, void *stream)
{
	int n = mwf_gpu_device_count();
	if (device < 0 || device >= n) return nullptr;
	if (hipSetDevice(device) != hipSuccess) return nullptr;
	mwf_gpu_t *g = new mwf_gpu_t();
	g->device = device;
	hipDeviceProp_t prop;
	if (hipGetDeviceProperties(&prop, device) != hipSuccess) { delete g; return nullptr; }
	g->n_cu = prop.multiProcessorCount;
	g->total_mem = prop.totalGlobalMem;
	if (stream) g->stream = (hipStream_t)stream;
	else {
		if (hipStreamCreateWithFlags(&g->stream, hipStreamNonBlocking) != hipSuccess) { delete g; return nullptr; }
		g->own_stream = true;
	}
	(void)hipEventCreate(&g->ev0);
	(void)hipEventCreate(&g->ev1);
	if (ensure(g, g->queue, kQueueInts * 4) || hipMemsetAsync(g->queue.p, 0, kQueueInts * 4, g->stream) != hipSuccess) {
		mwf_gpu_destroy(g);
		return nullptr;
	}
	return g;
}

static void trim(mwf_gpu_t *g)
{
	(void)hipStreamSynchronize(g->stream);
	for (DevBuf *b : {&g->ring, &g->sring, &g->good, &g->tb, &g->row_off, &g->row_lo, &g->cig_scratch, &g->snap, &g->snap_meta, &g->seg, &g->dbg,
	                  &g->coop_edge, &g->coop_misc, &g->sys_box, &g->sys_prog, &g->sys_log, &g->sys_ep, &g->sys_park, &g->sys_ring, &g->sys_sring, &g->sys_good, &g->retry_ids,
	                  &g->spare_block, &g->spare_cig})
		release(g, *b);
	g->dev_bytes_peak = g->dev_bytes;
}

void mwf_gpu_destroy(mwf_gpu_t *g)
{
	if (!g) return;
	(void)hipSetDevice(g->device);
	trim(g);
	release(g, g->queue);
	if (g->pin) (void)hipHostFree(g->pin);
	if (g->res_pin) (void)hipHostFree(g->res_pin);
	for (hipEvent_t e : {g->ev0, g->ev1, g->pin_ev[0], g->pin_ev[1]})
		if (e) (void)hipEventDestroy(e);
	if (g->own_stream) (void)hipStreamDestroy(g->stream);
	delete g;
}

const char *mwf_gpu_last_error(const mwf_gpu_t *g) { return g ? g->err.c_str() : "no engine (no gfx950 device could be opened)"; }

int mwf_gpu_set(mwf_gpu_t *g, const char *name, int64_t value)
{
	if (!g || !name) return -1;
	if (!strcmp(name, "tb_budget_mb")) g->tb_budget_mb = value;
	else if (!strcmp(name, "lowmem_budget_mb")) g->lowmem_budget_mb = std::max<int64_t>(0, value);
	else if (!strcmp(name, "coop_min_len")) g->coop_min_len = value;
	else if (!strcmp(name, "seq2bit")) g->seq2bit = (int)value;
	else if (!strcmp(name, "ring16")) g->ring16 = (int)value;
	else if (!strcmp(name, "band_span") && value >= 0 && value <= 2) g->band_span = (int)value;
	else if (!strcmp(name, "wide_slots") && (value == 0 || value == 3 || value == 4)) g->wide_slots = (int)value;
	else if (!strcmp(name, "lane_max_len")) g->lane_max_len = (int)std::max<int64_t>(0, std::min<int64_t>(value, 8000));
	else if (!strcmp(name, "mid_max_pairs")) g->mid_max_pairs = (int)std::max<int64_t>(-1, std::min<int64_t>(value, 1 << 20));
	else if (!strcmp(name, "host_results")) g->res_pin_on = value != 0;
	else if (!strcmp(name, "div_aware")) g->div_aware = value != 0;
	else if (!strcmp(name, "dev_retry")) g->dev_retry = value != 0;
	else if (!strcmp(name, "band_fold")) g->band_fold = value != 0;
	else if (!strcmp(name, "trim")) { (void)hipSetDevice(g->device); trim(g); }
	else return -1;
	++g->tun_gen;
	return 0;
}

int mwf_gpu_test_hook(mwf_gpu_t *g, const char *name, int64_t value)
{
	if (!g || !name) return -1;
	if (!strcmp(name, "block")) {
		if (value != 0 && value != 64 && value != 128 && value != 256 && value != 512 && value != 768 && value != 1024) return -1;
		g->block = (int)value;
	} else if (!strcmp(name, "force_kind")) g->force_kind = (int)value;
	else if (!strcmp(name, "band_pack")) g->band_pack = (int)value;
	else if (!strcmp(name, "lane_chunks") && value >= 0 && value <= 4) g->lane_chunks = (int)value;
	else if (!strcmp(name, "mid_block") && (value == 0 || value == 256 || value == 512 || value == 1024)) g->mid_block = (int)value;
	else if (!strcmp(name, "lds_e2")) g->lds_e2 = value != 0;
	else if (!strcmp(name, "scalar_generic")) g->scalar_generic = value != 0;
	else if (!strcmp(name, "coop_spin_limit")) g->coop_spin_limit = std::max<int64_t>(0, std::min<int64_t>(value, 0x7fffffff));
	else if (!strcmp(name, "coop_tb_cap_mb")) g->coop_tb_cap = std::max<int64_t>(1, value) << 20;
	else if (!strcmp(name, "coop_grid")) g->coop_grid_cap = (int)std::max<int64_t>(0, value);
	else if (!strcmp(name, "sys_p") && sys_p_supported((int)value)) g->sys_p = (int)value;
	else if (!strcmp(name, "sys_c") && (value == 0 || sys_c_supported((int)value))) g->sys_c = (int)value;
	else if (!strcmp(name, "work_order") && value >= 0 && value <= 3) g->work_order = (int)value;
	else if (!strcmp(name, "timeline")) g->timeline = (int64_t*)(intptr_t)value;
	else return -1;
	++g->tun_gen;
	return 0;
}

void mwf_gpu_get_stats(const mwf_gpu_t *g, mwf_gpu_stats_t *st)
{
	if (!g || !st) return;
	mwf_gpu_t *m = const_cast<mwf_gpu_t*>(g);
	if (m->ev_pending) {
		(void)hipSetDevice(m->device);
		float ms = 0;
		if (hipEventSynchronize(m->ev1) == hipSuccess && hipEventElapsedTime(&ms, m->ev0, m->ev1) == hipSuccess) m->stats.kernel_ms = ms;
		m->ev_pending = false;
	}
	m->stats.dev_bytes = m->dev_bytes, m->stats.dev_bytes_peak = m->dev_bytes_peak;
	*st = m->stats;
}


mwf_gpu_batch_t *mwf_gpu_batch_upload(mwf_gpu_t *g, int32_t n, const char *seqs, int64_t seq_bytes,
                                      const int64_t *t_off, const int32_t *tl, const int64_t *q_off, const int32_t *ql)
{
	if (!g || n < 0 || seq_bytes < 0) return nullptr;
	return batch_from_host(g, n, tl, nullptr, ql, nullptr, seqs, seq_bytes, t_off, q_off);
}

mwf_gpu_batch_t *mwf_gpu_batch_wrap(mwf_gpu_t *g, int32_t n, const void *d_seqs, int64_t seq_bytes,
                                    const int64_t *d_t_off, const int32_t *d_tl, const int64_t *d_q_off, const int32_t *d_ql,
                                    const int32_t *h_tl, const int32_t *h_ql)
{
	if (!g || n < 0) return nullptr;
	(void)hipSetDevice(g->device);
	BlockLayout L;
	mwf_gpu_batch_t *b = batch_common(g, n, h_tl, h_ql, 0, false, L);
	if (!b) return nullptr;
	b->d_seqs = (const uint8_t*)d_seqs, b->seq_bytes = seq_bytes;
	b->d_t_off = d_t_off, b->d_q_off = d_q_off, b->d_tl = d_tl, b->d_ql = d_ql;
	if (upload_segments(g, (char*)b->block.p, std::vector<Seg>{Seg{b->h_order.data(), (size_t)n * 4}})) {
		mwf_gpu_batch_free(b);
		return nullptr;
	}
	if (g->div_aware) b->div_est = estimate_divergence_device(g, b);
	return b;
}

void mwf_gpu_batch_free(mwf_gpu_batch_t *b)
{
	if (!b) return;
	mwf_gpu_t *g = b->g;
	(void)hipSetDevice(g->device);
	if (b->busy) (void)hipStreamSynchronize(g->stream);
	if (g->res_pin_owner == b) g->res_pin_owner = nullptr;
	give_block(g, g->spare_block, b->block);
	give_block(g, g->spare_cig, b->cig);
	for (DevBuf *d : {&b->ops_summary, &b->ops_map[0], &b->ops_map[1], &b->ops_map_off[0], &b->ops_map_off[1]}) release(g, *d);
	delete b;
}

}


extern "C" {

int mwf_gpu_batch_results(mwf_gpu_t *g, mwf_gpu_batch_t *b, int32_t *s, int64_t *n_iter, int32_t *n_cigar)
{
	if (!g || !b) return -1;
	(void)hipSetDevice(g->device);
	if (int rc = finalize(g, b)) return rc;
	const size_t n = (size_t)b->n;
	if (s && n) memcpy(s, b->h_s.data(), n * 4);
	if (n_iter && n) memcpy(n_iter, b->h_iter.data(), n * 8);
	if (n_cigar && n) memcpy(n_cigar, b->h_ncig.data(), n * 4);
	return 0;
}

const int32_t *mwf_gpu_batch_dev_scores(const mwf_gpu_batch_t *b) { return b ? b->d_s : nullptr; }
const int64_t *mwf_gpu_batch_dev_iters(const mwf_gpu_batch_t *b) { return b ? b->d_iter : nullptr; }
const int32_t *mwf_gpu_batch_dev_status(const mwf_gpu_batch_t *b) { return b ? b->d_status : nullptr; }

int32_t mwf_gpu_batch_cigar(mwf_gpu_t *g, mwf_gpu_batch_t *b, int32_t i, uint32_t *dst, int32_t cap)
{
	if (!g || !b || i < 0 || i >= b->n) return -1;
	(void)hipSetDevice(g->device);
	if (int rc = finalize(g, b)) return rc;
	const int32_t nc = b->h_ncig[i];
	if (nc > cap) return -5;
	if (nc <= 0) return nc;
	if (b->h_cig_valid) memcpy(dst, b->h_cig.data() + b->h_cigoff[i], (size_t)nc * 4);
	else HIP_TRY(g, hipMemcpy(dst, b->d_cig_pool + b->h_cigoff[i], (size_t)nc * 4, hipMemcpyDeviceToHost));
	return nc;
}

int mwf_gpu_batch_fetch_cigars(mwf_gpu_t *g, mwf_gpu_batch_t *b)
{
	if (!g || !b) return -1;
	(void)hipSetDevice(g->device);
	return fetch_cigars(g, b);
}


static int own_cigars(mwf_gpu_t *g, mwf_gpu_batch_t *b, const char *who)
{
	if (int rc = finalize(g, b)) return rc;
	if (!(b->opt.flag & MWF_F_CIGAR)) { g->err = std::string(who) + ": the batch's last align was score-only (no CIGARs to work on; align with MWF_F_CIGAR)"; return -2; }
	return 0;
}

static int ops_block(mwf_gpu_batch_t *b)
{
	if (b->ops_max_len < 0) {
		b->ops_max_len = 0;
		for (int32_t i = 0; i < b->n; ++i) b->ops_max_len = std::max<int64_t>(b->ops_max_len, (int64_t)b->h_tl[i] + b->h_ql[i]);
	}
	return cigar_ops_block(b->ops_max_len);
}

static CigarOpsArgs ops_args(const mwf_gpu_batch_t *b)
{
	CigarOpsArgs a{};
	a.seqs = b->d_seqs, a.t_off = b->d_t_off, a.q_off = b->d_q_off, a.tl = b->d_tl, a.ql = b->d_ql, a.n_pairs = b->n;
	a.words = b->d_cig_pool, a.word_off = b->d_cigoff, a.n_words = b->d_ncig, a.status = b->d_status;
	return a;
}

int mwf_gpu_batch_dev_cigars(mwf_gpu_t *g, mwf_gpu_batch_t *b, const uint32_t **pool, const int64_t **word_off, const int32_t **n_words, int64_t *pool_words)
{
	if (!g || !b) return -1;
	(void)hipSetDevice(g->device);
	if (int rc = own_cigars(g, b, "mwf_gpu_batch_dev_cigars")) return rc;
	if (pool) *pool = b->d_cig_pool;
	if (word_off) *word_off = b->d_cigoff;
	if (n_words) *n_words = b->d_ncig;
	if (pool_words) *pool_words = b->n > 0 ? b->cig_used : 0;
	return 0;
}

int mwf_gpu_batch_summarize(mwf_gpu_t *g, mwf_gpu_batch_t *b, const mwf_opt_t *opt, const uint32_t *d_words, const int64_t *d_word_off, const int32_t *d_n_words)
{
	if (!g || !b) return -1;
	(void)hipSetDevice(g->device);
	const bool own = !d_words && !d_word_off && !d_n_words;
	if (!own && (!d_words || !d_word_off || !d_n_words)) { g->err = "mwf_gpu_batch_summarize: foreign CIGARs need all three device arrays (words, offsets, counts)"; return -2; }
	if (own) { if (int rc = own_cigars(g, b, "mwf_gpu_batch_summarize")) return rc; }
	else if (b->busy) HIP_TRY(g, hipStreamSynchronize(g->stream));
	if (!opt && !b->aligned) { g->err = "mwf_gpu_batch_summarize: opt == NULL needs an earlier align of the batch"; return -2; }
	const mwf_opt_t &o = opt ? *opt : b->opt;
	b->summary_valid = false;
	if (b->n == 0) { b->summary_valid = true; return 0; }
	if (ensure(g, b->ops_summary, (size_t)b->n * sizeof(mwf_aln_summary_t))) return -1;
	CigarOpsArgs a = ops_args(b);
	if (!own) a.words = d_words, a.word_off = d_word_off, a.n_words = d_n_words, a.status = nullptr;
	a.x = o.x, a.o1 = o.o1, a.e1 = o.e1, a.o2 = o.o2, a.e2 = o.e2;
	a.mode = 0, a.summary = (int32_t*)b->ops_summary.p;
	if (launch_cigar_ops(a, ops_block(b), g->stream)) { g->err = "kernel launch failed (CIGAR summary)"; return -1; }
	b->summary_valid = true;
	return 0;
}

const mwf_aln_summary_t *mwf_gpu_batch_dev_summary(const mwf_gpu_batch_t *b)
{
	return b && b->summary_valid ? (const mwf_aln_summary_t*)b->ops_summary.p : nullptr;
}

int mwf_gpu_batch_summary(mwf_gpu_t *g, mwf_gpu_batch_t *b, mwf_aln_summary_t *host_out)
{
	if (!g || !b || !host_out) return -1;
	(void)hipSetDevice(g->device);
	if (!b->summary_valid) { g->err = "mwf_gpu_batch_summary: no summary (call mwf_gpu_batch_summarize after the align)"; return -2; }
	return download(g, host_out, b->ops_summary.p, (size_t)b->n * sizeof(mwf_aln_summary_t));
}

int mwf_gpu_batch_map(mwf_gpu_t *g, mwf_gpu_batch_t *b, int32_t which)
{
	if (!g || !b || which < 0 || which > 1) return -1;
	(void)hipSetDevice(g->device);
	if (int rc = own_cigars(g, b, "mwf_gpu_batch_map")) return rc;
	b->map_valid[which] = false;
	std::vector<int64_t> &off = b->h_map_off[which];
	if (off.empty()) {
		off.assign((size_t)b->n + 1, 0);
		for (int32_t i = 0; i < b->n; ++i) off[i + 1] = off[i] + (which == 0 ? b->h_ql[i] : b->h_tl[i]);
	}
	if (b->n == 0) { b->map_valid[which] = true; return 0; }
	if (ensure(g, b->ops_map[which], std::max<size_t>((size_t)off[b->n] * 4, 256))) return -1;
	if (!b->map_off_uploaded[which]) {
		if (ensure(g, b->ops_map_off[which], ((size_t)b->n + 1) * 8)) return -1;
		if (upload_segments(g, (char*)b->ops_map_off[which].p, std::vector<Seg>{Seg{off.data(), ((size_t)b->n + 1) * 8}})) return -1;
		b->map_off_uploaded[which] = true;
	}
	CigarOpsArgs a = ops_args(b);
	a.mode = 1 + which, a.map = (int32_t*)b->ops_map[which].p, a.map_off = (const int64_t*)b->ops_map_off[which].p;
	if (launch_cigar_ops(a, ops_block(b), g->stream)) { g->err = "kernel launch failed (coordinate map)"; return -1; }
	b->map_valid[which] = true;
	return 0;
}

const int32_t *mwf_gpu_batch_dev_map(const mwf_gpu_batch_t *b, int32_t which)
{
	return b && which >= 0 && which <= 1 && b->map_valid[which] ? (const int32_t*)b->ops_map[which].p : nullptr;
}

int mwf_gpu_batch_map_fetch(mwf_gpu_t *g, mwf_gpu_batch_t *b, int32_t which, int32_t *host_out, int64_t *host_off)
{
	if (!g || !b || which < 0 || which > 1) return -1;
	(void)hipSetDevice(g->device);
	if (!b->map_valid[which]) { g->err = "mwf_gpu_batch_map_fetch: no map (call mwf_gpu_batch_map after the align)"; return -2; }
	const std::vector<int64_t> &off = b->h_map_off[which];
	if (host_off) memcpy(host_off, off.data(), off.size() * 8);
	if (!host_out || b->n == 0) { HIP_TRY(g, hipStreamSynchronize(g->stream)); return 0; }
	return download(g, host_out, b->ops_map[which].p, (size_t)off[b->n] * 4);
}

int32_t mwf_gpu_debug_band(mwf_gpu_t *g, mwf_gpu_batch_t *b, const mwf_opt_t *opt, int32_t pair, int32_t *lohi, int32_t cap)
{
	if (!g || !b) return -1;
	b->debug_pair = pair;
	int rc = mwf_gpu_batch_align(g, b, opt);
	if (rc == 0) rc = finalize(g, b);
	b->debug_pair = -1;
	if (rc) return rc;
	const int32_t n = std::min<int32_t>(cap, std::max(0, b->h_s[pair] >= 0 ? b->h_s[pair] : 0));
	if (n > 0) HIP_TRY(g, hipMemcpy(lohi, g->dbg.p, (size_t)n * 8, hipMemcpyDeviceToHost));
	return n;
}

int mwf_gpu_test_pair_sketch(mwf_gpu_t *g, mwf_gpu_batch_t *b, int32_t *hits)
{
	if (!g || !b || !hits) return -1;
	(void)hipSetDevice(g->device);
	if (b->busy) HIP_TRY(g, hipStreamSynchronize(g->stream));
	if (b->n == 0) return 0;
	if (launch_pair_sketch(b->d_seqs, b->d_t_off, b->d_tl, b->d_q_off, b->d_ql, nullptr, b->n, b->d_dbg4, g->stream)) { g->err = "kernel launch failed (pair sketch)"; return -1; }
	HIP_TRY(g, hipMemcpyAsync(hits, b->d_dbg4, (size_t)b->n * 4, hipMemcpyDeviceToHost, g->stream));
	HIP_TRY(g, hipStreamSynchronize(g->stream));
	return 0;
}


void mwf_opt_init(mwf_opt_t *opt)
{
	memset(opt, 0, sizeof(*opt));
	opt->x = 4;
	opt->o1 = 4, opt->e1 = 2;
	opt->o2 = 15, opt->e2 = 1;
	opt->kmer = 13, opt->max_occ = 2, opt->min_len = 30;
}

}

namespace {

struct EnginePool {
	std::mutex mu;
	std::vector<mwf_gpu_t*> idle[kMaxDevices];
};
EnginePool &engine_pool() { static EnginePool *p = new EnginePool(); return *p; }

mwf_gpu_t *acquire_engine(int dev)
{
	if (dev < 0 || dev >= kMaxDevices || dev >= mwf_gpu_device_count()) {
		char what[192];
		snprintf(what, sizeof(what), "device ordinal %d (MWF_DEVICE / devices[]) is not one of the %d visible gfx950 devices; this library has no CPU path", dev, mwf_gpu_device_count());
		fatal(what, nullptr);
	}
	EnginePool &P = engine_pool();
	{
		std::lock_guard<std::mutex> lock(P.mu);
		std::vector<mwf_gpu_t*> &v = P.idle[dev];
		if (!v.empty()) {
			mwf_gpu_t *g = v.back();
			v.pop_back();
			return g;
		}
	}
	mwf_gpu_t *g = mwf_gpu_create(dev, nullptr);
	if (!g) fatal("cannot open a HIP device; this library has no CPU path", nullptr);
	return g;
}

void release_engine(mwf_gpu_t *g)
{
	EnginePool &P = engine_pool();
	std::lock_guard<std::mutex> lock(P.mu);
	P.idle[g->device % kMaxDevices].push_back(g);
}

int parse_ordinal(const char *e)
{
	if (!e || !*e) return -1;
	char *end = nullptr;
	const long v = strtol(e, &end, 10);
	return (*end == 0 && v >= 0 && v < 1 << 20) ? (int)v : -1;
}

// ... 180 lines not shown
```

miniwfa_amd/csrc/mwf_engine.h:

```cpp
#pragma once
#include <hip/hip_runtime.h>
#include <algorithm>
#include <cstdio>
#include <cstdlib>
#include <cstring>
#include <map>
#include <mutex>
#include <shared_mutex>
#include <numeric>
#include <string>
#include <chrono>
#include <cmath>
#include <functional>
#include <thread>
#include <vector>
#include "miniwfa.h"
#include "kalloc.h"
#include "mwf_internal.h"

namespace mwf {
namespace host {


[[noreturn]] inline void fatal(const char *what, const char *detail)
{
	fprintf(stderr, "[libmwf_hip] fatal: %s%s%s\n", what, detail ? ": " : "", detail ? detail : "");
	abort();
}

struct DevBuf {
	void *p = nullptr;
	size_t bytes = 0;
};

constexpr size_t kPinHalfMax = (size_t)16 << 20;
constexpr int kCigBlock = 256, kCigBlockGrid = 8192, kCigBlockPairs = 4096;
constexpr int kQueueSlots = 64;
constexpr int kLaneCounters = 64, kLaneStride = 32, kLaneSets = 4, kQueueInts = kQueueSlots + kLaneSets * kLaneCounters * kLaneStride;
constexpr int kMaxDevices = 64;

inline size_t align_up(size_t v, size_t a) { return (v + a - 1) / a * a; }


}
}

using namespace mwf;
using namespace mwf::host;


struct mwf_gpu_s {
	int device = 0;
	hipStream_t stream = nullptr;
	bool own_stream = false;
	int n_cu = 0;
	size_t total_mem = 0;
	std::string err;
	int block = 0;
	bool dev_retry = true;
	int retry_mode = 0;
	int retry_slot = 0;
	bool band_fold = true;
	bool div_aware = true;
	int64_t tun_gen = 0;
	int64_t coop_min_len = 0;
	int64_t tb_budget_mb = 0;
	int force_kind = -1;
	int work_order = 1;
	int64_t *timeline = nullptr;
	int res_pin_on = 1;
	int lane_chunks = 0;
	int lane_max_len = 325;
	int mid_max_pairs = -1;
	int mid_block = 0;
	int band_pack = -1;
	int wide_slots = 0;
	int band_span = 1;
	int ring16 = 1;
	bool ring16_off_once = false;
	int seq2bit = 1;
	bool acgt_off_once = false;
	int lds_e2 = 1;
	int scalar_generic = 0;
	int64_t coop_spin_limit = 1 << 23;
	int64_t coop_tb_cap = (int64_t)96 << 30;
	int64_t coop_tb_mult = 1;
	int64_t lowmem_budget_mb = 0;
	int sys_p = 8;
	int sys_c = 0;
	DevBuf ring, sring, good, tb, row_off, row_lo, cig_scratch, snap, snap_meta, seg, queue, dbg, coop_edge, coop_misc;
	DevBuf retry_ids;
	DevBuf sys_box, sys_prog, sys_log, sys_ep, sys_park, sys_ring, sys_sring, sys_good;
	DevBuf spare_block, spare_cig;
	int queue_next = 0;
	int lane_set_next = 0;
	bool queue_clean = false;
	void *pin = nullptr;
	size_t pin_half = 0;
	hipEvent_t pin_ev[2] = {nullptr, nullptr};
	void *res_pin = nullptr;
	const void *res_pin_owner = nullptr;
	bool pin_busy[2] = {false, false};
	hipEvent_t ev0 = nullptr, ev1 = nullptr;
	bool ev_pending = false;
	mwf_gpu_stats_t stats{};
	int64_t dev_bytes = 0, dev_bytes_peak = 0;
	std::map<uint64_t, int> occ_cache;
	int coop_grid = -1;
	int coop_grid_cap = 0;
};

struct mwf_gpu_batch_s {
	mwf_gpu_t *g = nullptr;
	int32_t n = 0;
	bool owns_inputs = false;
	DevBuf block;
	const uint8_t *d_seqs = nullptr;
	int64_t seq_bytes = 0;
	const int64_t *d_t_off = nullptr, *d_q_off = nullptr;
	const int32_t *d_tl = nullptr, *d_ql = nullptr;
	std::vector<int32_t> h_tl, h_ql;
	int64_t max_seq_lds = 0;
	int64_t max_tl = 0;
	int32_t *d_order = nullptr;
	std::vector<int32_t> h_order;
	std::vector<int32_t> h_len_order;
	std::vector<int8_t> h_class;
	std::vector<int8_t> h_kind;
	float div_est = 0;
	std::vector<int8_t> h_acgt;
	std::vector<int8_t> h_flags;
	unsigned long long *d_cig_head = nullptr;
	int32_t *d_status = nullptr, *d_s = nullptr, *d_ncig = nullptr, *d_dbg4 = nullptr;
	int64_t *d_iter = nullptr, *d_cigoff = nullptr, *d_cells1 = nullptr;
	size_t out_off = 0, out_bytes = 0;
	bool out_in_pin = false;
	bool results_preinit = false;
	DevBuf cig;
	uint32_t *d_cig_pool = nullptr;
	int64_t cig_pool_words = 0;
	int32_t cig_block = 0;
	bool aligned = false, finalized = false, busy = false;
	mwf_opt_t opt{};
	std::vector<int32_t> h_s, h_ncig, h_status;
	std::vector<int64_t> h_iter, h_cigoff, h_cells1;
	int64_t cig_used = 0;
	int32_t cig_block_left = 0;
	std::vector<uint32_t> h_cig;
	bool h_cig_valid = false;
	struct PlanCache {
		bool valid = false;
		int32_t opt_key[8] = {0, 0, 0, 0, 0, 0, 0, 0};
		int64_t tun_key[14] = {0, 0, 0, 0, 0, 0, 0, 0, 0, 0, 0, 0, 0, 0};
		int64_t max_len = 0, max_bound = 0;
		bool has_groups = false, mid_bytes = false;
		int8_t wide_state = 0;
		bool wide_measured = false;
		struct GI { int32_t n = 0; int64_t max_len = 0, max_bound = 0, max_bound1 = 0, max_tl = 0, max_seq_lds = 0, max_exp_win = 0; } gi[15];
		std::vector<int8_t> cls0, flags0;
	} plan;
	std::vector<char> host_out;
	size_t out_bytes_score = 0;
	int32_t last_grid = 0, n_retries = 0;
	int32_t *d_retry_ids = nullptr;
	bool dev_retry_used = false;
	int32_t debug_pair = -1;
	DevBuf ops_summary, ops_map[2], ops_map_off[2];
	bool summary_valid = false, map_valid[2] = {false, false};
	std::vector<int64_t> h_map_off[2];
	bool map_off_uploaded[2] = {false, false};
	int64_t ops_max_len = -1;
};


#define HIP_TRY(g, call)                                                              \
	do {                                                                              \
		hipError_t e_ = (call);                                                       \
		if (e_ != hipSuccess) {                                                       \
			(g)->err = std::string(#call) + ": " + hipGetErrorString(e_);             \
			return -1;                                                                \
		}                                                                             \
	} while (0)

namespace mwf {
namespace host {

void account(mwf_gpu_t *g, int64_t delta);
int ensure(mwf_gpu_t *g, DevBuf &b, size_t bytes);
void release(mwf_gpu_t *g, DevBuf &b);
int take_block(mwf_gpu_t *g, DevBuf &spare, DevBuf &out, size_t bytes);
void give_block(mwf_gpu_t *g, DevBuf &spare, DevBuf &b);
int pin_reserve(mwf_gpu_t *g, size_t half);
struct Seg { const void *src; size_t len; };
int upload_segments(mwf_gpu_t *g, char *dst, const std::vector<Seg> &segs);
int download(mwf_gpu_t *g, void *dst, const void *src, size_t bytes);
struct BlockLayout {
	size_t order = 0, t_off = 0, q_off = 0, tl = 0, ql = 0, seqs = 0, in_end = 0;
	size_t head = 0, status = 0, s = 0, ncig = 0, iter = 0, cigoff = 0, cells1 = 0, score_end = 0, out_end = 0, dbg4 = 0, retry = 0, total = 0;
};
constexpr int kRetryCap = 256;
constexpr int kRetrySlots = 2;
BlockLayout layout_block(size_t n, size_t seq_bytes, bool owned);
mwf_gpu_batch_t *batch_common(mwf_gpu_t *g, int32_t n, const int32_t *h_tl, const int32_t *h_ql, size_t seq_bytes, bool owned, BlockLayout &L);
mwf_gpu_batch_t *batch_from_host(mwf_gpu_t *g, int32_t n, const int32_t *tl, const char *const *ts, const int32_t *ql, const char *const *qs,
                                 const char *packed, int64_t packed_bytes, const int64_t *p_t_off, const int64_t *p_q_off);
float estimate_divergence_device(mwf_gpu_t *g, mwf_gpu_batch_t *b);
double sketch_divergence(int32_t hit, int32_t tot, int32_t lt);
extern "C" int mwf_gpu_test_hook(mwf_gpu_t *g, const char *name, int64_t value);
int64_t coalesce_window_us();
void exact_coalesced(void *km, const mwf_opt_t *opt, int32_t tl, const char *ts, int32_t ql, const char *qs, mwf_rst_t *r);

Penalty make_penalty(const mwf_opt_t &o);
const char *validate(const mwf_opt_t &o);
int64_t penalty_bound(const mwf_opt_t &o, int64_t tl, int64_t ql, bool honour_max_s);
int coop_grid_limit(mwf_gpu_t *g);
int finalize(mwf_gpu_t *g, mwf_gpu_batch_t *b);
int fetch_cigars(mwf_gpu_t *g, mwf_gpu_batch_t *b);

}
}
```

miniwfa_amd/csrc/mwf_internal.h:

```cpp
#pragma once
#include <stdint.h>

namespace mwf {

constexpr int32_t kNegInf = -0x40000000;
constexpr int32_t kMaxRing = 256;
constexpr int32_t kBigRing = 4096;

enum : int32_t {
	ST_OK = 0,
	ST_STOPPED = 1,
	ST_TB_OVERFLOW = 2,
	ST_ROWS_OVERFLOW = 3,
	ST_CIGAR_OVERFLOW = 4,
	ST_SNAP_OVERFLOW = 5,
	ST_INTERNAL = 6,
	ST_PENDING = 7,
	ST_BAND_OVERFLOW = 8,
	ST_ALPHABET = 9
};

struct Penalty {
	int32_t x;
	int32_t oe1;
	int32_t e1;
	int32_t oe2;
	int32_t e2;
	int32_t o1, o2;
	int32_t nH;
	int32_t n1;
	int32_t n2;
};

struct BatchArgs {
	const uint8_t *seqs;
	const int64_t *t_off, *q_off;
	const int32_t *tl, *ql;
	const int32_t *order;
	int32_t n_pairs;
	int32_t *queue;
	int32_t queue_parts;
	Penalty pen;
	int32_t want_cigar;
	int32_t step;
	int32_t max_s;
	int64_t max_iter;
	int32_t debug_pair;
	int32_t *ring;
	int32_t *sring;
	int64_t ring_slot_ints;
	int32_t W;
	unsigned long long *good;
	int32_t GW;
	uint8_t *tb;
	int64_t tb_slot_bytes;
	int64_t *row_off;
	int32_t *row_lo;
	int64_t rows_slot;
	uint32_t *cig_scratch;
	int64_t cig_scratch_slot;
	uint32_t *cig_pool;
	unsigned long long *cig_head;
	int64_t cig_pool_words;
	int32_t *snap;
	int64_t snap_slot_ints;
	int32_t *snap_meta;
	int64_t snap_meta_slot;
	int32_t *seg;
	int64_t seg_slot;
	int32_t *out_s;
	int64_t *out_iter;
	int32_t *out_ncig;
	int64_t *out_cigoff;
	int32_t *out_status;
	int64_t *out_cells1;
	int32_t *out_dbg;
	int32_t *dbg;
	int32_t dbg_cap;
	int32_t coop_pair;
	int32_t lds_e2_cols;
	int32_t ring16;
	int32_t scalar_generic;
	int32_t band_lds_seq;
	int32_t band_fold;
	int32_t coop_groups, coop_group_size;
	int64_t coop_edge_stride;
	int64_t coop_sedge_off;
	int64_t coop_misc_stride;
	const int32_t *coop_pair_ids;
	uint32_t coop_spin_limit;
	int32_t *retry_ids;
	unsigned int *retry_count;
	int32_t retry_cap;
	const unsigned int *n_pairs_dev;
	int32_t coop_pass;
	int32_t *coop_edge;
	int32_t *coop_flags;
	unsigned int *coop_sync;
	int32_t *coop_state;
	int32_t sys_p;
	int32_t sys_c;
	int32_t sys_spread;
	int32_t *sys_box;
	int64_t sys_box_stride;
	unsigned long long *sys_prog;
	int64_t sys_prog_stride;
	int32_t *sys_log;
	int64_t sys_log_stride;
	int32_t *sys_park;
	int64_t sys_park_stride;
	int64_t *sys_ep;
	int64_t sys_ep_stride;
	int32_t report_wide;
	int32_t cig_block;
	int32_t lane_chunks;
	int32_t sys_coop_launch;
	int64_t *timeline;
};

int launch_reset(int32_t *status, int32_t *s, int32_t n, unsigned long long *cig_head, int32_t *queue, int32_t n_queue, void *stream);
int launch_batch(const BatchArgs &a, int grid, int block, void *stream);
int launch_sketch(const uint8_t *seqs, const int64_t *t_off, const int32_t *tl, const int64_t *q_off, const int32_t *ql, int32_t n, int32_t samples, int32_t *out, void *stream);
int launch_pair_sketch(const uint8_t *seqs, const int64_t *t_off, const int32_t *tl, const int64_t *q_off, const int32_t *ql, const int32_t *order, int32_t n, int32_t *out, void *stream);
struct CigarOpsArgs {
	const uint8_t *seqs;
	const int64_t *t_off, *q_off;
	const int32_t *tl, *ql;
	int32_t n_pairs;
	const uint32_t *words;
	const int64_t *word_off;
	const int32_t *n_words;
	const int32_t *status;
	int32_t x, o1, e1, o2, e2;
	int32_t mode;
	int32_t *summary;
	int32_t *map;
	const int64_t *map_off;
};
int cigar_ops_block(int64_t max_len);
int launch_cigar_ops(const CigarOpsArgs &a, int block, void *stream);
int  bigring_kernel_occupancy();
int  batch_kernel_occupancy(int block, bool stream_pass, int lds_e2_cols, bool ring16);

struct BandGeom {
	int block;
	int packed;
	int span;
	int lds_bytes;
	int seq2;
	int lane;
};
bool coop_supported(const Penalty &p);
int64_t coop_chunk_slots(int grid);
int64_t sys_chunk_slots(int grid);
int  sys_owned_cols(int p, int c);
bool sys_c_supported(int c);
bool sys_p_supported(int p);
constexpr int64_t sys_box_ints(int p, int nef, bool seg) { return ((seg ? 4 : 2) * p * (p + nef) + 2 * p + 31) / 32 * 32; }
constexpr int64_t sys_park_ints(int nef, bool seg) { return (int64_t)(seg ? 2 : 1) * nef * 64 * 4; }
constexpr int kSysNotResident = -3;
int  sys_max_grid();
int  launch_sys_pass(const BatchArgs &a, int grid, void *stream);
int  launch_sys_pass_deep(const BatchArgs &a, int grid, void *stream);
int  launch_sys_walk(const BatchArgs &a, void *stream);
int  launch_sys_trace(const BatchArgs &a, void *stream);
int  launch_sys_finish(const BatchArgs &a, void *stream);

bool lane_supported(const Penalty &p);
int  lane_lds_bytes(const Penalty &p, int chunks, int64_t seq_bytes);
int  launch_lane(const BatchArgs &a, int grid, int lds, bool seq2, void *stream);
int  lane_kernel_occupancy(int lds, bool cigar);

bool mid_supported(const Penalty &p);
int  mid_lds_bytes(const Penalty &p, int groups, int64_t seq_bytes);
int  launch_mid(const BatchArgs &a, int grid, int block, int lds, bool seq2, void *stream);

bool band2_supported(const Penalty &p);
int  launch_band2(const BatchArgs &a, int grid, const BandGeom &g, void *stream);
int  band2_kernel_occupancy(const Penalty &p, const BandGeom &g, bool cigar);
bool band2_biased512_supported(const Penalty &p);
int  band2_biased512_chunks();
int  band2_span_chunks();

}
```

miniwfa_amd/csrc/mwf_plan.cpp:

```cpp
#include "mwf_engine.h"

namespace mwf {
namespace host {


Penalty make_penalty(const mwf_opt_t &o)
{
	Penalty p;
	p.x = o.x, p.o1 = o.o1, p.o2 = o.o2, p.e1 = o.e1, p.e2 = o.e2;
	p.oe1 = o.o1 + o.e1, p.oe2 = o.o2 + o.e2;
	int32_t mp = std::max(p.x, std::max(p.oe1, p.oe2));
	p.nH = mp + 1, p.n1 = p.e1 + 1, p.n2 = p.e2 + 1;
	return p;
}

const char *validate(const mwf_opt_t &o)
{
	if (o.x < 1 || o.e1 < 1 || o.e2 < 1) return "x, e1 and e2 must be >= 1 (a zero lag would make a wavefront depend on itself)";
	if (o.o1 < 0 || o.o2 < 0) return "gap-open penalties must be >= 0";
	if (std::max<int64_t>(o.x, std::max<int64_t>((int64_t)o.o1 + o.e1, (int64_t)o.o2 + o.e2)) + 1 > kBigRing) return "max(x, o1+e1, o2+e2) must be < 4096";
	if (o.step < 0) return "step must be >= 0";
	return nullptr;
}

int64_t penalty_bound(const mwf_opt_t &o, int64_t tl, int64_t ql, bool honour_max_s)
{
	auto gap = [&](int64_t L) -> int64_t { return L == 0 ? 0 : std::min<int64_t>(o.o1 + L * o.e1, o.o2 + L * o.e2); };
	int64_t b = gap(tl) + gap(ql);
	if (honour_max_s && o.max_s > 0) b = std::min<int64_t>(b, (int64_t)o.max_s + 1);
	return b;
}

constexpr int64_t kBandMicroWindow = (1 * 3 - 1) * 256 - 64, kBandTinyWindow = (2 * 3 - 1) * 256 - 64, kBandSmallWindow = (4 * 3 - 1) * 256 - 64;
constexpr int64_t kBandWideWindow = (8 * 3 - 1) * 256 - 64;
constexpr int64_t kBandWide4Window = (8 * 4 - 1) * 256 - 64;
constexpr int64_t kBandSpanMaxSeq = 62000;
inline int64_t band_span_window() { return ((int64_t)band2_span_chunks() - 1) * 256 - 64; }

struct Plan {
	int kind = 0;
	BandGeom band{0, 0, 0, 0, 0, 0};
	int block = 256, grid = 1;
	int32_t W = 0, GW = 0;
	int64_t ring_slot_ints = 0, rows_slot = 0, tb_slot_bytes = 0, cig_scratch_slot = 0;
	int64_t snap_slot_ints = 0, snap_meta_slot = 0, seg_slot = 0;
	bool low_mem = false, cigar = false;
};

int cached_occupancy(mwf_gpu_t *g, const Penalty &P, const Plan &pl, int lds_e2_cols, bool stream_pass, bool ring16 = false);

void choose_kernel(mwf_gpu_t *g, const mwf_opt_t &opt, const Penalty &P, int64_t max_len, int64_t max_bound,
                   int64_t max_seq_lds, int64_t max_tl, int want_kind, Plan &pl, int geom_block = 0, int64_t window_hint = 0)
{
	pl.kind = 0;
	const bool low_mem = (opt.flag & MWF_F_CIGAR) && opt.step > 0;
	const bool can_packed = band2_supported(P) && g->band_pack != 0;
	if (geom_block == 32 && want_kind != 0 && !low_mem && lane_supported(P)) {
		const int chunks = g->lane_chunks > 0 ? g->lane_chunks : max_len <= 400 ? 3 : 4;
		BandGeom lg{64, 1, 64 * chunks, lane_lds_bytes(P, chunks, max_seq_lds), (g->seq2bit != 0 && !g->acgt_off_once && max_len >= 450) ? 1 : 0, 1};
		if (lg.lds_bytes <= 60 * 1024) {
			pl.kind = 2, pl.band = lg;
			return;
		}
	}
	if (geom_block == 33 && want_kind != 0 && !low_mem && mid_supported(P)) {
		const int64_t want_cols = (std::min<int64_t>(max_len + 1, 2 * max_bound + 3) + 2 * P.nH + 63) / 64 * 64;
		int groups = (int)std::min<int64_t>(want_cols / 64, 128);
		while (groups > 1 && mid_lds_bytes(P, groups, max_seq_lds) > 158 * 1024) --groups;
		const int lds = mid_lds_bytes(P, groups, max_seq_lds);
		if (lds <= 158 * 1024) {
			const int64_t by_len = window_hint > 0 ? std::max<int64_t>(max_len, window_hint * 100 / 28) : max_len;
			const int block = g->mid_block ? g->mid_block : (by_len <= 1000 ? 256 : by_len <= 2500 ? 512 : 1024);
			const int seq2 = g->seq2bit != 0 && !g->acgt_off_once;
			pl.kind = 2, pl.band = BandGeom{block, 1, 64 * groups, lds, seq2, 2};
			return;
		}
	}
	if (want_kind == 0 || low_mem || !can_packed) return;
	if (geom_block == 514) {
		const int64_t need_lds = ((max_len >> 4) + 4) * 4;
		if (g->seq2bit == 0 || g->acgt_off_once || need_lds > 70 * 1024 || !band2_biased512_supported(P)) return;
		const bool six = max_len + 1 > 7 * (int64_t)(band2_biased512_chunks() * 256) / 2 || (window_hint > 0 && window_hint + 768 > ((int64_t)band2_biased512_chunks() - 1) * 256 - 64);
		const int chunks = band2_biased512_chunks() + (six ? 8 : 0);
		pl.kind = 2, pl.band = BandGeom{512, 2, chunks * 256, (int)((need_lds + 15) / 16 * 16), 1, 0};
		pl.cigar = (opt.flag & MWF_F_CIGAR) != 0;
		if (cached_occupancy(g, P, pl, 0, false) >= 2) return;
		pl.kind = 0, pl.band = BandGeom{0, 0, 0, 0, 0, 0}, geom_block = 1024;
	}
	if (geom_block == 1024) {
		const int64_t need_lds = ((max_len >> 4) + 4) * 4;
		if (g->band_span == 0 || g->seq2bit == 0 || g->acgt_off_once || need_lds > 150 * 1024) return;
		pl.kind = 2, pl.band = BandGeom{1024, 1, (int)band2_span_chunks() * 256, (int)((need_lds + 15) / 16 * 16), 1, 0};
		return;
	}
	const int64_t max_window = window_hint > 0 ? std::min<int64_t>(std::min<int64_t>(max_len + 1, 2 * max_bound + 3), window_hint) : std::min<int64_t>(max_len + 1, 2 * max_bound + 3);
	BandGeom bg;
	bg.packed = 0, bg.seq2 = 0, bg.lane = 0;
	const bool range_ok = max_tl + max_bound < 32767;
	if (!range_ok) return;
	bg.packed = 1;
	bg.block = max_window <= kBandMicroWindow ? 64 : max_window <= kBandTinyWindow ? 128 : max_window <= kBandSmallWindow ? 256 : 512;
	if (g->block == 64 || g->block == 128 || g->block == 256 || g->block == 512 || g->block == 768) bg.block = g->block;
	if (g->block == 0 && (geom_block == 64 || geom_block == 128 || geom_block == 256)) bg.block = geom_block;
	bg.span = bg.block / 64 * (bg.block != 768 ? 3 : 2) * 256;
	const bool four_slots = bg.block == 512 && g->block == 0 && window_hint > kBandWideWindow && window_hint <= kBandWide4Window;
	if (four_slots) bg.span = 512 / 64 * 4 * 256;
	if (want_kind != 2 && max_len + 1 > 4 * (int64_t)bg.span) return;
	const int64_t lds_cap = bg.block >= 768 ? 140 * 1024 : bg.block >= 512 ? 70 * 1024 : bg.block == 256 ? 36 * 1024 : bg.block == 128 ? 18 * 1024 : 9 * 1024;
	const bool seq2 = g->seq2bit != 0 && !g->acgt_off_once;
	const int64_t need_lds = seq2 ? ((max_len >> 4) + 4) * 4 : max_seq_lds;
	bg.lds_bytes = need_lds <= lds_cap ? (int)((need_lds + 15) / 16 * 16) : 0;
	bg.seq2 = seq2 && bg.lds_bytes > 0;
	if (bg.block == 768) bg.seq2 = 0, bg.lds_bytes = max_seq_lds <= 140 * 1024 ? (int)((max_seq_lds + 15) / 16 * 16) : 0;
	else if (!bg.seq2) {
		bg.block = 768, bg.span = 768 / 64 * 2 * 256;
		bg.lds_bytes = max_seq_lds <= 140 * 1024 ? (int)((max_seq_lds + 15) / 16 * 16) : 0;
	}
	if (bg.lds_bytes == 0) return;
	pl.kind = 2, pl.band = bg;
}

int cached_occupancy(mwf_gpu_t *g, const Penalty &P, const Plan &pl, int lds_e2_cols, bool stream_pass, bool ring16)
{
	uint64_t key;
	if (pl.kind == 2)
		key = 1ull | (uint64_t)pl.band.block << 4 | (uint64_t)(pl.band.packed == 1) << 16 | (uint64_t)(pl.band.packed == 2) << 15 | (uint64_t)(pl.band.lds_bytes > 0) << 17 | (uint64_t)pl.cigar << 18 |
		      (uint64_t)(pl.band.seq2 != 0) << 3 | (uint64_t)(pl.band.lane == 1) << 2 | (uint64_t)(pl.band.block == 512 && pl.band.span > 6144) << 1 | (uint64_t)(pl.band.block == 512 ? pl.band.span / 2048 : 0) << 56 | (uint64_t)(pl.band.lane == 2) << 19 | (uint64_t)P.e1 << 20 | (uint64_t)P.e2 << 28 | (uint64_t)pl.band.lds_bytes << 36;
	else key = 2ull | (uint64_t)pl.block << 4 | (uint64_t)stream_pass << 16 | (uint64_t)ring16 << 17 | (uint64_t)(P.nH > kMaxRing) << 18 | (uint64_t)lds_e2_cols << 20;
	auto it = g->occ_cache.find(key);
	if (it != g->occ_cache.end()) return it->second;
	const int per = pl.kind == 2 && pl.band.lane == 2 ? 1
	              : pl.kind == 2 && pl.band.lane ? lane_kernel_occupancy(pl.band.lds_bytes, pl.cigar)
	              : pl.kind == 2 ? band2_kernel_occupancy(P, pl.band, pl.cigar)
	              : P.nH > kMaxRing ? bigring_kernel_occupancy()
	                             : batch_kernel_occupancy(pl.block, stream_pass, lds_e2_cols, ring16);
	g->occ_cache[key] = per;
	return per;
}

int64_t tb_budget_bytes(mwf_gpu_t *g)
{
	if (g->tb_budget_mb > 0) return g->tb_budget_mb << 20;
	size_t fr = 0, tot = 0;
	if (hipMemGetInfo(&fr, &tot) != hipSuccess) fr = (size_t)8 << 30, tot = fr;
	int64_t b = (int64_t)(fr / 5 * 4) + (int64_t)g->tb.bytes;
	return std::min<int64_t>(b, std::min<int64_t>((int64_t)64 << 30, (int64_t)(tot / 4)));
}

std::shared_mutex g_dev_gate[kMaxDevices];

int run_batch_kernel(mwf_gpu_t *g, mwf_gpu_batch_t *b, const mwf_opt_t &opt, const int32_t *d_order, int32_t n_items,
                     int slots, int64_t max_len, int64_t max_bound, int64_t max_bound1, bool timed,
                     int want_kind, int64_t max_tl, int64_t max_seq_lds, int timed_end, int geom_block, int *ran_kind, int64_t window_hint = 0)
{
	const Penalty P = make_penalty(opt);
	Plan pl;
	pl.cigar = (opt.flag & MWF_F_CIGAR) != 0;
	pl.low_mem = pl.cigar && opt.step > 0;
	pl.block = g->block > 0 && g->block != 768 ? g->block : (std::min<int64_t>(max_len + 1, 2 * max_bound + 3) >= 8192 ? 512 : 256);
	choose_kernel(g, opt, P, max_len, max_bound, max_seq_lds, max_tl, want_kind >= 0 ? want_kind : g->force_kind, pl, geom_block, window_hint);
	int per_cu, lds_e2_cols = 0;
	bool ring16 = false;
	if (pl.kind == 2) {
		pl.block = pl.band.block;
		per_cu = cached_occupancy(g, P, pl, 0, false);
	} else {
		if (g->lds_e2 && pl.block == 512 && g->block == 0 && P.e2 == 1 && !g->scalar_generic && !pl.low_mem && P.nH <= kMaxRing) {
			lds_e2_cols = 16384;
			const int64_t s_guess = b->div_est > 0 && g->div_aware ? (int64_t)(6.9 * b->div_est * (double)max_tl) + 256 : max_len / 8;
			ring16 = g->ring16 != 0 && !g->ring16_off_once && max_tl + std::max<int64_t>(s_guess, max_len / 8) < 65500;
			pl.block = ring16 ? (pl.cigar ? 768 : 512) : 768;
		}
		if (P.nH > kMaxRing) pl.block = 256;
		per_cu = cached_occupancy(g, P, pl, lds_e2_cols, !g->scalar_generic, ring16);
	}
	slots = std::max(1, std::min(slots, g->n_cu * std::max(1, per_cu)));
	if (P.nH > kMaxRing) {
		const int64_t per_slot = (int64_t)(P.nH + 2 * P.n1 + 2 * P.n2) * ((max_len + 3 + 255) / 256 * 256 + 512) * 4 * (pl.low_mem ? 2 : 1);
		slots = (int)std::max<int64_t>(1, std::min<int64_t>(slots, (int64_t)(g->total_mem / 10) / std::max<int64_t>(per_slot, 1)));
	}
	if (getenv("MWF_DEBUG"))
		fprintf(stderr, "[libmwf_hip] kernel kind %d: block %d packed %d lds %d B, %d workgroup(s) per CU, %d slots, %d pairs\n", pl.kind, pl.block,
		        pl.band.packed, pl.band.lds_bytes, per_cu, slots, n_items);
	pl.grid = std::max(1, std::min<int>(slots, n_items));
	pl.W = (int32_t)((max_len + 3 + 255) / 256 * 256 + 512);
	pl.GW = pl.W / 64 + 2;
	pl.ring_slot_ints = (int64_t)(P.nH + 2 * P.n1 + 2 * P.n2) * pl.W;
	if (pl.kind == 2 && pl.band.lane) pl.ring_slot_ints = 64;
	const size_t S = (size_t)pl.grid;

	if (ensure(g, g->ring, S * pl.ring_slot_ints * 4)) return -1;
	if (ensure(g, g->good, S * (size_t)P.nH * pl.GW * 8)) return -1;
	if (pl.cigar) {
		pl.rows_slot = max_bound + 2;
		pl.cig_scratch_slot = max_len + 2;
		int64_t worst = (max_bound + 1) * (max_len + 1);
		if (pl.low_mem && opt.step > 2 * P.nH) {
			worst = std::min(worst, (max_bound + 1) * std::min<int64_t>(max_len + 1, 2 * (int64_t)(opt.step + 2 * P.nH) + 8));
		}
		worst += 8 * (max_bound + 2);
		if (pl.kind == 2 && pl.band.lane == 1) worst = (std::min<int64_t>(max_bound, 256) + 2) * pl.band.span;
		if (pl.kind == 2 && pl.band.lane == 2) worst = (max_bound + 2) * pl.band.span;
		int64_t per = worst;
		if ((int64_t)g->tb.bytes < (int64_t)S * worst || g->tb_budget_mb > 0) per = std::min(per, std::max<int64_t>(tb_budget_bytes(g), (int64_t)g->tb.bytes) / (int64_t)S);
		if (g->tb_budget_mb > 0) per = std::min(per, (g->tb_budget_mb << 20) / (int64_t)S);
		pl.tb_slot_bytes = std::max<int64_t>(4096, per) / 4 * 4;
		if (ensure(g, g->tb, S * (size_t)pl.tb_slot_bytes)) return -1;
		if (ensure(g, g->row_off, S * (size_t)pl.rows_slot * 8)) return -1;
		if (ensure(g, g->row_lo, S * (size_t)pl.rows_slot * 4)) return -1;
		if (ensure(g, g->cig_scratch, S * (size_t)pl.cig_scratch_slot * 4)) return -1;
	}
	if (pl.low_mem) {
		const int64_t NS = P.nH + 2 * P.n1 + 2 * P.n2;
		const int64_t n_snap_max = max_bound1 / opt.step + 2;
		pl.seg_slot = n_snap_max;
		pl.snap_meta_slot = n_snap_max * (4 + 4 * NS);
		int64_t worst = 0;
		for (int64_t j = 1; j <= n_snap_max; ++j)
			worst += NS * std::min<int64_t>(max_len + 1, 2 * j * opt.step + 3);
		const int64_t budget = (int64_t)(std::max<int64_t>(tb_budget_bytes(g), (int64_t)g->snap.bytes) / 4 / (int64_t)S);
		pl.snap_slot_ints = std::max<int64_t>(1024, std::min(worst, budget));
		if (ensure(g, g->sring, S * pl.ring_slot_ints * 4)) return -1;
		if (ensure(g, g->snap, S * (size_t)pl.snap_slot_ints * 4)) return -1;
		if (ensure(g, g->snap_meta, S * (size_t)pl.snap_meta_slot * 4)) return -1;
		if (ensure(g, g->seg, S * (size_t)pl.seg_slot * 8)) return -1;
	}

	BatchArgs a;
	memset(&a, 0, sizeof(a));
	a.seqs = b->d_seqs, a.t_off = b->d_t_off, a.q_off = b->d_q_off, a.tl = b->d_tl, a.ql = b->d_ql;
	a.order = d_order, a.n_pairs = n_items;
	a.timeline = g->timeline;
	if (pl.kind == 2 && pl.band.lane == 1 && n_items > pl.grid) {
		a.queue_parts = kLaneCounters;
		if (g->queue_clean && g->lane_set_next < kLaneSets) a.queue = (int32_t*)g->queue.p + kQueueSlots + (g->lane_set_next++) * kLaneCounters * kLaneStride;
		else {
			a.queue = (int32_t*)g->queue.p + kQueueSlots;
			HIP_TRY(g, hipMemsetAsync(a.queue, 0, (size_t)kLaneCounters * kLaneStride * 4, g->stream));
		}
	} else if (pl.kind == 2 && pl.band.lane == 1) a.queue = nullptr;
	else if (pl.kind == 2 && (pl.band.lane || pl.band.packed) && n_items <= pl.grid && !g->queue_clean) a.queue = nullptr;
	else if (g->queue_clean && g->queue_next < kQueueSlots) a.queue = (int32_t*)g->queue.p + g->queue_next++;
	else {
		a.queue = (int32_t*)g->queue.p;
		HIP_TRY(g, hipMemsetAsync(g->queue.p, 0, 4, g->stream));
	}
	if (g->retry_mode == 1) a.retry_ids = b->d_retry_ids + g->retry_slot * kRetryCap, a.retry_cap = kRetryCap, a.retry_count = (unsigned int*)(b->d_cig_head + 2 + g->retry_slot);
	if (g->retry_mode == 2) a.n_pairs_dev = (const unsigned int*)(b->d_cig_head + 2 + g->retry_slot), a.queue = nullptr, a.queue_parts = 0;
	a.scalar_generic = g->scalar_generic;
	a.band_fold = g->band_fold ? 1 : 0;
	a.lds_e2_cols = lds_e2_cols;
	a.ring16 = ring16 ? 1 : 0;
	a.lane_chunks = pl.kind == 2 && pl.band.lane ? pl.band.span / 64 : 0;
	a.pen = P;
	a.want_cigar = pl.cigar ? 1 : 0;
	a.step = pl.low_mem ? opt.step : 0;
	a.max_s = opt.max_s, a.max_iter = opt.max_iter;
	a.debug_pair = b->debug_pair;
	a.ring = (int32_t*)g->ring.p;
	a.sring = pl.low_mem ? (int32_t*)g->sring.p : nullptr;
	a.ring_slot_ints = pl.ring_slot_ints, a.W = pl.W;
	a.good = (unsigned long long*)g->good.p, a.GW = pl.GW;
	a.tb = pl.cigar ? (uint8_t*)g->tb.p : nullptr, a.tb_slot_bytes = pl.tb_slot_bytes;
	a.row_off = pl.cigar ? (int64_t*)g->row_off.p : nullptr;
	a.row_lo = pl.cigar ? (int32_t*)g->row_lo.p : nullptr;
	a.rows_slot = pl.rows_slot;
	a.cig_scratch = pl.cigar ? (uint32_t*)g->cig_scratch.p : nullptr, a.cig_scratch_slot = pl.cig_scratch_slot;
	a.cig_pool = b->d_cig_pool, a.cig_head = b->d_cig_head, a.cig_pool_words = b->cig_pool_words;
	a.cig_block = 0;
	if (b->cig_block > 0 && pl.grid <= b->cig_block_left) a.cig_block = b->cig_block, b->cig_block_left -= pl.grid;
	a.report_wide = geom_block == 0 && window_hint == kBandWide4Window ? 1 : 0;
	a.snap = pl.low_mem ? (int32_t*)g->snap.p : nullptr, a.snap_slot_ints = pl.snap_slot_ints;
	a.snap_meta = pl.low_mem ? (int32_t*)g->snap_meta.p : nullptr, a.snap_meta_slot = pl.snap_meta_slot;
	a.seg = pl.low_mem ? (int32_t*)g->seg.p : nullptr, a.seg_slot = pl.seg_slot;
	a.out_s = b->d_s, a.out_iter = b->d_iter, a.out_ncig = b->d_ncig, a.out_cigoff = b->d_cigoff;
	a.out_status = b->d_status, a.out_cells1 = b->d_cells1, a.out_dbg = b->d_dbg4;
	a.dbg = b->debug_pair >= 0 ? (int32_t*)g->dbg.p : nullptr;
	a.dbg_cap = b->debug_pair >= 0 ? (int32_t)(g->dbg.bytes / 8) : 0;

	if (timed) HIP_TRY(g, hipEventRecord(g->ev0, g->stream));
	std::shared_lock<std::shared_mutex> gate(g_dev_gate[g->device % kMaxDevices]);
	const int lrc = pl.kind == 2 && pl.band.lane == 2 ? launch_mid(a, pl.grid, pl.band.block, pl.band.lds_bytes, pl.band.seq2 != 0, g->stream)
	              : pl.kind == 2 && pl.band.lane ? launch_lane(a, pl.grid, pl.band.lds_bytes, pl.band.seq2 != 0, g->stream)
	              : pl.kind == 2 ? launch_band2(a, pl.grid, pl.band, g->stream)
	                             : launch_batch(a, pl.grid, pl.block, g->stream);
	gate.unlock();
	if (lrc != 0) {
		g->err = "kernel launch failed";
		return -1;
	}
	b->last_grid = std::max(b->last_grid, pl.grid);
	if (timed_end < 0 ? timed : timed_end != 0) {
		HIP_TRY(g, hipEventRecord(g->ev1, g->stream));
		g->ev_pending = true;
	}
	g->stats.n_launches += 1;
	g->stats.grid = std::max(g->stats.grid, pl.grid), g->stats.block = pl.block, g->stats.kernel_kind = pl.kind;
	g->stats.packed = pl.kind == 2 ? (pl.band.lane == 2 ? 33 : pl.band.lane ? 32 : (pl.band.packed ? 1 : 0)) : (ring16 ? 16 : 0);
	g->stats.lowmem_two_pass = pl.low_mem ? 1 : 0;
	if (ran_kind) *ran_kind = pl.kind;
	return 0;
}



int coop_grid_limit(mwf_gpu_t *g)
{
	if (g->coop_grid < 0) g->coop_grid = std::min(sys_max_grid(), g->n_cu);
	return g->coop_grid_cap > 0 ? std::min(g->coop_grid, g->coop_grid_cap) : g->coop_grid;
}

int coop_group_size(int n_cu, int64_t len, bool alone, int ow = 256)
{
	int G = n_cu;
	const int64_t chunks = alone ? len / ow + (ow == 256 ? 3 : 8) : len / ow / 3 + (ow == 256 ? 8 : 12);
	while (G > (alone ? 64 : 16) && chunks <= coop_chunk_slots(G / 2)) G /= 2;
	return G;
}

int run_coop_group(mwf_gpu_t *g, mwf_gpu_batch_t *b, const mwf_opt_t &opt, const std::vector<int32_t> &pairs, int Gs, bool first, bool last)
{
	const Penalty P = make_penalty(opt);
	const bool cigar = (opt.flag & MWF_F_CIGAR) != 0, low_mem = cigar && opt.step > 0;
	const int n_groups = (int)pairs.size();
	if (n_groups < 1 || Gs < 1 || (int64_t)Gs * n_groups > coop_grid_limit(g)) { g->err = "whole-device kernel cannot be made resident"; return -1; }
	int64_t len = 0, bound = 0, bound1 = 0;
	bool traced = false;
	for (int32_t pair : pairs) {
		len = std::max<int64_t>(len, (int64_t)b->h_tl[pair] + b->h_ql[pair]);
		bound = std::max(bound, penalty_bound(opt, b->h_tl[pair], b->h_ql[pair], true));
		bound1 = std::max(bound1, penalty_bound(opt, b->h_tl[pair], b->h_ql[pair], false));
		traced |= b->debug_pair == pair;
	}
	const int32_t W = (int32_t)((len + 3 + 255) / 256 * 256 + 512), GW = W / 64 + 2;
	const int64_t TC = coop_chunk_slots(Gs);
	const size_t NG = (size_t)n_groups;
	const bool use_sys = true;
	const int sysP = g->sys_p, sysP2 = g->sys_p;
	auto window_cap = [&](int c) -> int64_t { return (TC - 4) * (int64_t)sys_owned_cols(sysP, c) - 2 * (257 + sysP); };
	bool wide_again = false;
	for (int32_t pair : pairs) wide_again |= (b->h_flags[pair] & 16) != 0;
	const int64_t est1 = std::min<int64_t>(len + 1, std::max<int64_t>(8192, b->div_est > 0 && g->div_aware ? (int64_t)(6.5 * b->div_est * (double)len) : len / 5));
	const int64_t est2 = std::min<int64_t>(len + 1, 2 * ((int64_t)opt.step + 2 * P.nH) + 8);
	const int c_first = g->sys_c ? g->sys_c : (!wide_again && est1 <= window_cap(1)) ? 1 : 4;
	const int c_second = g->sys_c ? g->sys_c : (!wide_again && est2 <= window_cap(1)) ? 1 : 4;
	bool two_pass = false;
	if (low_mem) {
		const int64_t budget = g->lowmem_budget_mb > 0 ? g->lowmem_budget_mb << 20 : (int64_t)8 << 30;
		two_pass = std::max<int64_t>((int64_t)1 << 30, 6000 * len) * (int64_t)NG * g->coop_tb_mult * (c_first == 1 ? 12 : 9) / 8 > budget;
	}
	const size_t gran_bytes = 4096;
	const size_t flag_ring_bytes = 0;
	const size_t misc_bytes = 4096 + flag_ring_bytes;
	if (ensure(g, g->coop_edge, NG * gran_bytes)) return -1;
	if (ensure(g, g->coop_misc, NG * misc_bytes + 4096)) return -1;
	int64_t rows_slot = 0, tb_bytes = 0, cig_scratch = 0, seg_slot = 0;
	if (cigar) {
		rows_slot = std::max(bound, bound1) + 2;
		cig_scratch = len + 2;
		const int64_t worst = NG * (rows_slot + 1) * (len + 8);
		int64_t guess = std::min<int64_t>(g->coop_tb_cap, std::max<int64_t>((int64_t)1 << 30, 6000 * len) * (int64_t)NG);
		if (two_pass) guess = std::min<int64_t>(guess, std::max<int64_t>((int64_t)64 << 20, (len * 3 / 100 + 1024) * std::min<int64_t>(len + 1, 2 * (int64_t)(opt.step + 2 * P.nH) + 8)) * (int64_t)NG);
		const int64_t lay = (two_pass ? c_second : c_first) == 1 ? 12 : (two_pass ? c_second : c_first) == 2 ? 10 : 9;
		const int64_t ep_guess = (len * 3 / 100 + 1024) / 256 + 2;
		if (use_sys) guess = std::min<int64_t>(g->coop_tb_cap, guess / 8 * lay + ep_guess * 8 * 65536 * (int64_t)NG);
		int64_t want = std::min(use_sys ? worst / 8 * lay + (rows_slot / 256 + 2) * 8 * 65536 * (int64_t)NG : worst, g->tb_budget_mb > 0 ? (g->tb_budget_mb << 20) : guess * g->coop_tb_mult);
		if ((int64_t)g->tb.bytes >= want) want = (int64_t)g->tb.bytes;
		else {
			size_t fr = 0, tot = 0;
			if (hipMemGetInfo(&fr, &tot) != hipSuccess) fr = (size_t)8 << 30;
			want = std::min<int64_t>(want, (int64_t)(fr / 10 * 9) + (int64_t)g->tb.bytes);
		}
		tb_bytes = std::max<int64_t>(4096, want / (int64_t)NG) / 4 * 4;
		if (ensure(g, g->row_off, NG * (size_t)rows_slot * 8)) return -1;
		if (ensure(g, g->row_lo, NG * (size_t)rows_slot * 4)) return -1;
		if (ensure(g, g->cig_scratch, NG * (size_t)cig_scratch * 4)) return -1;
		if (low_mem) {
			seg_slot = bound1 / opt.step + 2;
			if (ensure(g, g->seg, NG * (size_t)seg_slot * 8)) return -1;
		}
		if (ensure(g, g->tb, NG * (size_t)tb_bytes)) return -1;
	}
	int64_t snap_slot_ints = 0, snap_meta_slot = 0;
	if (two_pass) {
		const int64_t NS = P.nH + 2 * P.e1 + 2 * P.e2, s_guess = len * 3 / 100 + 1024, n_guess = s_guess / opt.step + 2;
		int64_t cols = 0;
		for (int64_t j = 1; j <= n_guess; ++j) cols += std::min<int64_t>(len + 1, 2 * j * opt.step) + 1100;
		snap_meta_slot = (bound1 / opt.step + 256 / opt.step + 4) * 8;
		snap_slot_ints = std::min<int64_t>(std::max<int64_t>((int64_t)4 << 20, NS * cols) * g->coop_tb_mult, ((int64_t)48 << 30) / 4) / 4 * 4;
		if (ensure(g, g->sys_sring, NG * (size_t)TC * P.nH * 256 * 4)) return -1;
		if (ensure(g, g->snap, NG * (size_t)snap_slot_ints * 4)) return -1;
		if (ensure(g, g->snap_meta, NG * (size_t)snap_meta_slot * 4)) return -1;
	}
	if (traced) {
		if (ensure(g, g->dbg, (size_t)8 * (bound + 2))) return -1;
		HIP_TRY(g, hipMemsetAsync(g->dbg.p, 0, g->dbg.bytes, g->stream));
	}

	const int64_t sys_rows = std::max(bound, bound1) + 2, sys_log_ints = 2 * (sys_rows + 256 + 8), sys_ep_words = 2 * (sys_rows / 256 + 3);
	const int sys_nef = 2 * P.e1 + 2 * P.e2;
	const int64_t sys_box_group = TC * 2 * std::max(sys_box_ints(sysP, sys_nef, two_pass), sys_box_ints(sysP2, sys_nef, false)), sys_park_group = TC * sys_park_ints(sys_nef, two_pass);
	if (use_sys) {
		if (ensure(g, g->sys_ring, NG * (size_t)TC * P.nH * 256 * 4)) return -1;
		if (ensure(g, g->sys_good, NG * (size_t)P.nH * TC * 4 * 8)) return -1;
		if (ensure(g, g->sys_box, NG * (size_t)sys_box_group * 4)) return -1;
		if (ensure(g, g->sys_prog, NG * (size_t)TC * 64)) return -1;
		if (ensure(g, g->sys_log, NG * (size_t)sys_log_ints * 4)) return -1;
		if (ensure(g, g->sys_ep, NG * (size_t)sys_ep_words * 8)) return -1;
		if (ensure(g, g->sys_park, NG * (size_t)sys_park_group * 4)) return -1;
	}
	BatchArgs a;
	memset(&a, 0, sizeof(a));
	a.seqs = b->d_seqs, a.t_off = b->d_t_off, a.q_off = b->d_q_off, a.tl = b->d_tl, a.ql = b->d_ql;
	a.n_pairs = b->n;
	a.pen = P;
	a.want_cigar = cigar ? 1 : 0;
	a.step = low_mem ? opt.step : 0;
	a.max_s = opt.max_s, a.max_iter = opt.max_iter;
	a.debug_pair = b->debug_pair;
	a.ring = (int32_t*)g->ring.p, a.ring_slot_ints = (int64_t)P.nH * W, a.W = W;
	a.good = (unsigned long long*)g->good.p, a.GW = GW;
	a.tb = cigar ? (uint8_t*)g->tb.p : nullptr, a.tb_slot_bytes = tb_bytes;
	a.row_off = cigar ? (int64_t*)g->row_off.p : nullptr, a.row_lo = cigar ? (int32_t*)g->row_lo.p : nullptr, a.rows_slot = rows_slot;
	a.cig_scratch = cigar ? (uint32_t*)g->cig_scratch.p : nullptr, a.cig_scratch_slot = cig_scratch;
	a.cig_pool = b->d_cig_pool, a.cig_head = b->d_cig_head, a.cig_pool_words = b->cig_pool_words;
	a.seg = low_mem ? (int32_t*)g->seg.p : nullptr, a.seg_slot = seg_slot;
	a.sring = two_pass ? (int32_t*)g->sys_sring.p : nullptr;
	a.snap = two_pass ? (int32_t*)g->snap.p : nullptr, a.snap_slot_ints = snap_slot_ints;
	a.snap_meta = two_pass ? (int32_t*)g->snap_meta.p : nullptr, a.snap_meta_slot = snap_meta_slot;
	a.out_s = b->d_s, a.out_iter = b->d_iter, a.out_ncig = b->d_ncig, a.out_cigoff = b->d_cigoff;
// ... 607 lines not shown
```

profiles/timing_probe_band2_chunk.py:

```python
import sys, os
sys.path.insert(0, os.path.dirname(os.path.dirname(os.path.abspath(__file__))))
import numpy as np
import miniwfa_amd as mw
from miniwfa_amd.api import lib
import ctypes as C
from miniwfa_amd.synth import synth_pair, PackedBatch
eng = mw.Engine(0)
if len(sys.argv) > 1: eng.set("band_fold", int(sys.argv[1]))
for n in (1, 512):
    b = eng.upload(PackedBatch([synth_pair(50000, 10000, 0.05)] * n))
    o = mw.opt_init()
    b.align(o); s = b.results()[0]
    cap = int(s[0])
    for wave in (0, 3, 7):
        o2 = mw.opt_init(max_iter=-(64 * wave) if wave else 0)
        buf = np.zeros(2 * cap, dtype=np.uint32)
        got = lib().mwf_gpu_debug_band(eng.h, b.h, C.byref(o2), 0, buf.ctypes.data, cap)
        a = buf[0:2 * got:2]; c = buf[1:2 * got:2]
        ph = np.stack([a & 0xfff, (a >> 12) & 0xfff, c & 0xfff, (c >> 12) & 0xfff, a >> 28], axis=1).astype(np.float64)
        q = ph[ph[:, 4] >= 1]
        print(f"pairs {n} wave {wave}: penalties with an active chunk {len(q)}: rows+recurrence {q[:,0].mean():.0f}, masks/liveness/geometry/edge stores {q[:,1].mean():.0f}, first probe {q[:,2].mean():.0f}, walks+store {q[:,3].mean():.0f}, sum {q[:,:4].sum(axis=1).mean():.0f}")
    b.free()
```

Baseline: 1.542 Gbp/s.

## Add LDS probe-table band2 kernel variant with 16-bit match lookups

Adds a separate band2 kernel build in which each block first builds a table of 16-bit, 8-base 2-bit sequence windows in LDS, one per position of target and query. The first match probe can then use a single ds_read_u16 per side instead of unaligned 64-bit word reads plus alignbit. The probe depth drops to 8 bases, so longer runs fall back to the wave-wide walk. The table costs extra LDS (about 2 bytes per base) and a build pass per pair. The planner enables it by default for 512-thread seq2 plans when occupancy stays at 2 or more blocks.

```diff
diff --git a/miniwfa_amd/build.py b/miniwfa_amd/build.py
--- a/miniwfa_amd/build.py
+++ b/miniwfa_amd/build.py
@@ -8,9 +8,9 @@
 ROOT = os.path.dirname(HERE)
 CSRC = os.path.join(HERE, "csrc")
 LIB = os.path.join(CSRC, "libmwf_hip.so")
-SOURCES = ["mwf_band2.hip", "mwf_band2_e3.hip", "mwf_band2_e4.hip", "mwf_band2_bi.hip", "mwf_band2_bi_deep.hip", "mwf_kernels.hip", "mwf_lane.hip", "mwf_mid.hip", "mwf_sys.hip", "mwf_sys_deep.hip", "mwf_cigar_ops.hip", "mwf_engine.cpp", "mwf_memory.cpp", "mwf_plan.cpp", "mwf_chain.cpp", "mwf_async.cpp", "kalloc.cpp", "mwf_dbg.cpp"]
+SOURCES = ["mwf_band2.hip", "mwf_band2_tab.hip", "mwf_band2_e3.hip", "mwf_band2_e4.hip", "mwf_band2_bi.hip", "mwf_band2_bi_deep.hip", "mwf_kernels.hip", "mwf_lane.hip", "mwf_mid.hip", "mwf_sys.hip", "mwf_sys_deep.hip", "mwf_cigar_ops.hip", "mwf_engine.cpp", "mwf_memory.cpp", "mwf_plan.cpp", "mwf_chain.cpp", "mwf_async.cpp", "kalloc.cpp", "mwf_dbg.cpp"]
 HEADERS = [os.path.join(CSRC, "mwf_internal.h"), os.path.join(CSRC, "mwf_device.h"), os.path.join(CSRC, "mwf_sys_pass.h"), os.path.join(CSRC, "mwf_engine.h"), os.path.join(ROOT, "include", "miniwfa.h"), os.path.join(ROOT, "include", "kalloc.h")]
-SOURCE_DEPS = {"mwf_band2_e3.hip": ["mwf_band2.hip"], "mwf_band2_e4.hip": ["mwf_band2.hip"], "mwf_band2_bi.hip": ["mwf_band2.hip"], "mwf_band2_bi_deep.hip": ["mwf_band2.hip"]}
+SOURCE_DEPS = {"mwf_band2_e3.hip": ["mwf_band2.hip"], "mwf_band2_e4.hip": ["mwf_band2.hip"], "mwf_band2_bi.hip": ["mwf_band2.hip"], "mwf_band2_bi_deep.hip": ["mwf_band2.hip"], "mwf_band2_tab.hip": ["mwf_band2.hip"]}
 
 
 def hipcc() -> str:
@@ -52,7 +52,7 @@
             print(" ".join(cmd))
         return cmd, subprocess.run(cmd, capture_output=True, text=True)
 
-    with ThreadPoolExecutor(max(1, min(6, len(jobs)))) as ex:
+    with ThreadPoolExecutor(max(1, min(7, len(jobs)))) as ex:
         for cmd, r in ex.map(run, jobs):
             if r.returncode != 0:
                 sys.stderr.write(r.stdout + r.stderr)
@@ -67,9 +67,9 @@
     return LIB
 
 
-KERNEL_FILES = {"wfa_band2_kernel": "mwf_band2.hip", "wfa_sys_kernel": "mwf_sys.hip", "wfa_sys_seg_kernel": "mwf_sys.hip", "wfa_batch_kernel": "mwf_kernels.hip",
+KERNEL_FILES = {"wfa_band2_kernel": "mwf_band2.hip", "wfa_band2_tab_kernel": "mwf_band2.hip", "wfa_sys_kernel": "mwf_sys.hip", "wfa_sys_seg_kernel": "mwf_sys.hip", "wfa_batch_kernel": "mwf_kernels.hip",
                 "wfa_lane_kernel": "mwf_lane.hip", "wfa_mid_kernel": "mwf_mid.hip"}
-KERNEL_HEADERS = {"mwf_sys.hip": ["mwf_sys_pass.h", "mwf_sys_deep.hip"], "mwf_band2.hip": ["mwf_band2_e3.hip", "mwf_band2_e4.hip", "mwf_band2_bi.hip", "mwf_band2_bi_deep.hip"]}
+KERNEL_HEADERS = {"mwf_sys.hip": ["mwf_sys_pass.h", "mwf_sys_deep.hip"], "mwf_band2.hip": ["mwf_band2_e3.hip", "mwf_band2_e4.hip", "mwf_band2_bi.hip", "mwf_band2_bi_deep.hip", "mwf_band2_tab.hip"]}
 
 
 def kernel_fingerprint(symbol: str) -> str | None:
diff --git a/miniwfa_amd/csrc/mwf_band2.hip b/miniwfa_amd/csrc/mwf_band2.hip
--- a/miniwfa_amd/csrc/mwf_band2.hip
+++ b/miniwfa_amd/csrc/mwf_band2.hip
@@ -22,6 +22,14 @@
 constexpr int kChunk = 256;
 constexpr int kFoldMaxLag = 8;
 constexpr int32_t kDeadPair = (int32_t)0x80008000u;
+#ifdef MWF_BAND2_TAB
+constexpr bool kTabProbe = true;
+#define MWF_BAND2_KERNEL wfa_band2_tab_kernel
+#else
+constexpr bool kTabProbe = false;
+#define MWF_BAND2_KERNEL wfa_band2_kernel
+#endif
+constexpr int kTabSlack = 258;
 
 __device__ __forceinline__ int32_t from_left(int32_t v, int32_t fill) { return __builtin_amdgcn_update_dpp(fill, v, 0x138, 0xf, 0xf, false); }
 __device__ __forceinline__ int32_t from_right(int32_t v, int32_t fill) { return __builtin_amdgcn_update_dpp(fill, v, 0x130, 0xf, 0xf, false); }
@@ -100,14 +108,14 @@
 {
 	return min(lead_eq2(__builtin_amdgcn_alignbit(p.t1, p.t0, (uint32_t)j << 1) ^ __builtin_amdgcn_alignbit(p.q1, p.q0, (uint32_t)iq << 1)), 17);
 }
-__device__ __forceinline__ int32_t run_wave16(int32_t qbase, int32_t j, int32_t iq, int32_t room, int32_t n0)
+__device__ __forceinline__ int32_t run_wave16(int32_t qbase, int32_t j, int32_t iq, int32_t room, int32_t n0, int32_t tbase = 0)
 {
 	const int32_t lane = threadIdx.x & 63;
 	int32_t n = n0;
 	while (n < room) {
 		const int32_t off = n + 16 * lane;
 		int32_t m = 0;
-		if (off < room) m = min(min(lead_eq2(seq16(0, j + off) ^ seq16(qbase, iq + off)), 16), room - off);
+		if (off < room) m = min(min(lead_eq2(seq16(tbase, j + off) ^ seq16(qbase, iq + off)), 16), room - off);
 		const unsigned long long stop = __ballot(m < 16);
 		if (stop == 0) { n += 1024; continue; }
 		const int32_t first = (int32_t)__builtin_ctzll(stop);
@@ -146,6 +154,19 @@
 		*(uint32_t*)(lds2 + base + 4 * w) = out;
 	}
 	return bad;
+}
+
+template <int T>
+__device__ __forceinline__ void build_probe_table(int32_t tl, int32_t ql, int32_t tbase, int32_t qbase)
+{
+	const int32_t n = tl + ql + kTabSlack;
+	for (int32_t e = threadIdx.x; e < n; e += T) {
+		const int32_t q = e - tl - 2;
+		uint32_t v = 0;
+		if (e <= tl) v = seq16(tbase, e);
+		else if (q >= 0 && q <= ql) v = seq16(qbase, q);
+		*(uint16_t*)(lds2 + 2 * e) = (uint16_t)v;
+	}
 }
 
 __device__ __forceinline__ uint32_t inm_bit(int32_t d, int32_t k, int32_t tl, int32_t ql)
@@ -231,7 +252,8 @@
 {
 	constexpr int NW = T / 64, NWK = NW * K, D = (E1 > E2 ? E1 : E2) + 1;
 	constexpr bool BI = is_span(T, K) || BI4;
-	constexpr int FULL = S2 ? 16 : 8;
+	constexpr bool TAB = kTabProbe && S2;
+	constexpr int FULL = TAB ? 8 : S2 ? 16 : 8;
 	constexpr int kAgeOut = FOLD ? kFoldMaxLag : D;
 	constexpr int kAge = (NWK + 2) * 16;
 	static_assert(D >= 2 && D <= 5, "edge-table ages");
@@ -284,7 +306,7 @@
 	}
 	__syncthreads();
 	if (tid < 64) {
-		const int32_t k0 = (S2 ? run_wave16(qoff, 0, 0, min(tl, ql), 0) : run_wave2(0, qoff, min(tl, ql), 0)) - 1;
+		const int32_t k0 = (S2 ? run_wave16(qoff, 0, 0, min(tl, ql), 0, TAB ? fresh(A).band_lds_tab : 0) : run_wave2(0, qoff, min(tl, ql), 0)) - 1;
 		if (tid == 0) {
 			const int32_t c = tl + 1, e = c & 3;
 			*(int16_t*)(Hb + 8 + (size_t)(uint32_t)(((c & ~3) + ((e & 1) << 1) + (e >> 1)) << 1)) = (int16_t)(k0 - B);
@@ -518,8 +540,9 @@
 			}
 			const int32_t cbp = both16(cb);
 			const int32_t xA = pk_sub(pk_sub(T0, cbp), RA);
-			const int32_t rjA = pk_minu(xA, TLp), rjB = pk_minu(pk_sub(xA, ONE), TLp);
-			const int32_t dA = pk_sub(pk_add(RA, cbp), TL1), dB = pk_add(dA, ONE);
+			const int32_t xAc = TAB ? pk_subsat(pk_subsat(T0, cbp), RA) : xA;
+			const int32_t rjA = pk_minu(xAc, TLp), rjB = pk_minu(TAB ? pk_subsat(xAc, ONE) : pk_sub(xA, ONE), TLp);
+			const int32_t dA = TAB ? pk_add(pk_add(RA, cbp), ONE) : pk_sub(pk_add(RA, cbp), TL1), dB = pk_add(dA, ONE);
 			const bool on_lo = kEpoch ? (cls & 2u) != 0 : g == ga, on_hi = kEpoch ? (cls & 4u) != 0 : g == gb;
 			const bool special = is_span(T, K) || (BI4 && !TB) || (kEpoch ? edgy : !inside || on_lo || on_hi) || track_good;
 			int32_t outA = 0, outB = 0;
@@ -594,7 +617,26 @@
 			const int32_t jA = pk_minu(pk_add(hA, ONEB), rjA), jB = pk_minu(pk_add(hB, ONEB), rjB);
 			const int32_t iqA = pk_add(jA, dA), iqB = pk_add(jB, dB);
 			int32_t cnt[4];
-			if (S2) {
+			if (TAB) {
+				uint32_t tv[4], qv[4];
+#pragma unroll
+				for (int u = 0; u < 4; ++u) {
+					const uint32_t J = (uint32_t)((u & 1) ? jB : jA), Q = (uint32_t)((u & 1) ? iqB : iqA);
+					uint32_t ta, qa;
+					if (u & 2) {
+						asm("v_add_u32_sdwa %0, %1, %1 dst_sel:DWORD dst_unused:UNUSED_PAD src0_sel:WORD_1 src1_sel:WORD_1" : "=v"(ta) : "v"(J));
+						asm("v_add_u32_sdwa %0, %1, %1 dst_sel:DWORD dst_unused:UNUSED_PAD src0_sel:WORD_1 src1_sel:WORD_1" : "=v"(qa) : "v"(Q));
+					} else {
+						asm("v_add_u32_sdwa %0, %1, %1 dst_sel:DWORD dst_unused:UNUSED_PAD src0_sel:WORD_0 src1_sel:WORD_0" : "=v"(ta) : "v"(J));
+						asm("v_add_u32_sdwa %0, %1, %1 dst_sel:DWORD dst_unused:UNUSED_PAD src0_sel:WORD_0 src1_sel:WORD_0" : "=v"(qa) : "v"(Q));
+					}
+					asm volatile("ds_read_u16 %0, %1" : "=v"(tv[u]) : "v"(ta));
+					asm volatile("ds_read_u16 %0, %1" : "=v"(qv[u]) : "v"(qa));
+				}
+				asm volatile("s_waitcnt lgkmcnt(0)" : "+v"(tv[0]), "+v"(tv[1]), "+v"(tv[2]), "+v"(tv[3]), "+v"(qv[0]), "+v"(qv[1]), "+v"(qv[2]), "+v"(qv[3]));
+#pragma unroll
+				for (int u = 0; u < 4; ++u) asm("v_ffbl_b32 %0, %1" : "=v"(cnt[u]) : "v"(tv[u] ^ qv[u]));
+			} else if (S2) {
 				uint64_t tw[4], qw[4];
 #pragma unroll
 				for (int u = 0; u < 4; ++u) {
@@ -629,8 +671,9 @@
 				}
 			}
 			typedef unsigned short us2_t __attribute__((ext_vector_type(2)));
-			const int32_t cA = MWF_BC(int32_t, (us2_t)__builtin_amdgcn_cvt_pk_u16((uint32_t)cnt[0], (uint32_t)cnt[2]));
-			const int32_t cB = MWF_BC(int32_t, (us2_t)__builtin_amdgcn_cvt_pk_u16((uint32_t)cnt[1], (uint32_t)cnt[3]));
+			int32_t cA = MWF_BC(int32_t, (us2_t)__builtin_amdgcn_cvt_pk_u16((uint32_t)cnt[0], (uint32_t)cnt[2]));
+			int32_t cB = MWF_BC(int32_t, (us2_t)__builtin_amdgcn_cvt_pk_u16((uint32_t)cnt[1], (uint32_t)cnt[3]));
+			if (TAB) cA = MWF_BC(int32_t, (us2_t)(MWF_BC(us2_t, cA) >> 1)), cB = MWF_BC(int32_t, (us2_t)(MWF_BC(us2_t, cB) >> 1));
 #if MWF_B2_TIMING == 2
 			if (timed) asm volatile("s_memtime %0\n\ts_waitcnt lgkmcnt(0)" : "=s"(tc3) : "v"(cA), "v"(cB) : "memory");
 #endif
@@ -639,6 +682,7 @@
 			int32_t nmA = pk_minu(m9A, FULLp), nmB = pk_minu(m9B, FULLp);
 			const int32_t pendp = pk_subsat(m9A, FULLp) | pk_subsat(m9B, FULLp);
 			if (__ballot(pendp != 0)) {
+				const int32_t tb0 = TAB ? fresh(A).band_lds_tab : 0;
 				int32_t hv[4] = {half_of(hA, 0) + B, half_of(hB, 0) + B, half_of(hA, 1) + B, half_of(hB, 1) + B};
 				int32_t nmat[4] = {(int32_t)((uint32_t)nmA & 0xffffu), (int32_t)((uint32_t)nmB & 0xffffu), (int32_t)((uint32_t)nmA >> 16), (int32_t)((uint32_t)nmB >> 16)};
 				const uint32_t pend = (uint32_t)(((uint32_t)m9A & 0xffffu) > (uint32_t)FULL) | (uint32_t)(((uint32_t)m9B & 0xffffu) > (uint32_t)FULL) << 1 |
@@ -653,7 +697,7 @@
 						for (int trip = 0; n < rm; ++trip) {
 							if (trip == 4) { open |= 1u << i; break; }
 							if (S2) {
-								const int32_t m = min(lead_eq2(seq16(0, j + n) ^ seq16(qoff, q + n)), 16);
+								const int32_t m = min(lead_eq2(seq16(tb0, j + n) ^ seq16(qoff, q + n)), 16);
 								n += m;
 								if (m < 16) break;
 							} else {
@@ -674,7 +718,7 @@
 						if (!((ob >> i) & 1u)) continue;
 						const int32_t hh = __builtin_amdgcn_readlane(hv[i], src);
 						const int32_t j = hh + 1, q = c0s + i - 1 - tl + j, rm = min(tl - j, ql - q);
-						const int32_t n = S2 ? run_wave16(qoff, j, q, rm, 80) : run_wave2(j, qoff + q, rm, 40);
+						const int32_t n = S2 ? run_wave16(qoff, j, q, rm, FULL + 64, tb0) : run_wave2(j, qoff + q, rm, 40);
 						nmat[i] = lane == src ? n : nmat[i];
 					}
 				}
@@ -813,7 +857,7 @@
 	return is_span(T, K) ? (T == 1024 ? 4 : 3) : T == 1024 ? 4 : T == kWideT ? kWideWaves : T <= 512 ? ((TB && T < 512) ? 3 : 4) : kWaves768;
 }
 template <int T, int K, int E1, int E2, bool TB, bool S2, bool BI4 = false, bool FOLD = false>
-__global__ __launch_bounds__(T, band2_waves(T, K, TB)) void wfa_band2_kernel(const BatchArgs)
+__global__ __launch_bounds__(T, band2_waves(T, K, TB)) void MWF_BAND2_KERNEL(const BatchArgs)
 {
 	constexpr int NWK = (T / 64) * K, D = (E1 > E2 ? E1 : E2) + 1;
 	KArgs &A0 = kernel_args();
@@ -835,15 +879,21 @@
 		const int32_t pair = A.order ? A.order[item] : item;
 		PairMem M;
 		pair_mem(A, (int32_t)blockIdx.x, pair, M);
-		const int32_t qoff = S2 ? ((M.tl >> 4) + 2) * 4 : ((M.tl + 3) & ~3) + 8;
+		constexpr bool TAB = kTabProbe && S2;
+		const int32_t toff = TAB ? A.band_lds_tab : 0;
+		const int32_t qoff = toff + (S2 ? ((M.tl >> 4) + 2) * 4 : ((M.tl + 3) & ~3) + 8);
 		PassResult R;
 		R.status = ST_OK, R.s = 0, R.info = 0, R.n_snap = 0, R.cells = 0;
 		if (S2) {
-			uint32_t bad = pack2bit<T>(M.ts, M.tl, 0);
+			uint32_t bad = pack2bit<T>(M.ts, M.tl, toff);
 			bad |= pack2bit<T>(M.qs, M.ql, qoff);
 			if (bad) sh.word[2] = 1;
 			__syncthreads();
 			if (uni(sh.word[2])) R.status = ST_ALPHABET;
+			if (TAB) {
+				if (2 * (M.tl + M.ql + kTabSlack) > toff) R.status = ST_BAND_OVERFLOW;
+				else if (R.status == ST_OK) build_probe_table<T>(M.tl, M.ql, toff, qoff);
+			}
 		} else {
 			for (int32_t j = threadIdx.x; j < M.tl; j += T) lds2[j] = M.ts[j];
 			for (int32_t j = threadIdx.x; j < M.ql; j += T) lds2[qoff + j] = M.qs[j];
@@ -853,7 +903,7 @@
 		if (R.status == ST_OK) R = band2_pass<T, K, E1, E2, TB, S2, BI4, FOLD>(A, M, sh, edge_base, qoff, trace);
 		if (T == 512 && K == 4 && R.n_snap && threadIdx.x == 0 && fresh(A0).report_wide) atomicOr((unsigned int*)(fresh(A0).cig_head + 1), 1u);
 		R.n_snap = 0;
-		if (S2) M.t2 = lds2, M.q2 = lds2 + qoff;
+		if (S2) M.t2 = lds2 + toff, M.q2 = lds2 + qoff;
 		if (TB && FOLD) M.tb_fwd = 1;
 		finish_pair(fresh(A0), M, (int32_t)blockIdx.x, pair, R, R.status, 0, T <= 256 ? &cig_loc : nullptr);
 	}
@@ -869,12 +919,12 @@
 		if (a.band_fold && a.pen.oe1 - a.pen.x == E1 && a.pen.oe1 < kFoldMaxLag) return launch_variant<T, K, E1, E2, TB, S2, BI4, true>(a, grid, lds, st);
 	}
 	if (lds > 48 * 1024) {
-		(void)hipFuncSetAttribute(reinterpret_cast<const void*>(&wfa_band2_kernel<T, K, E1, E2, TB, S2, BI4, FOLD>), hipFuncAttributeMaxDynamicSharedMemorySize, lds);
+		(void)hipFuncSetAttribute(reinterpret_cast<const void*>(&MWF_BAND2_KERNEL<T, K, E1, E2, TB, S2, BI4, FOLD>), hipFuncAttributeMaxDynamicSharedMemorySize, lds);
 		(void)hipGetLastError();
 	}
 	if (getenv("MWF_DEBUG"))
 		fprintf(stderr, "[libmwf_hip] band2 launch: T %d K %d E1 %d E2 %d TB %d S2 %d BI4 %d FOLD %d, %d pairs, grid %d\n", T, K, E1, E2, (int)TB, (int)S2, (int)BI4, (int)FOLD, (int)a.n_pairs, grid);
-	hipLaunchKernelGGL((wfa_band2_kernel<T, K, E1, E2, TB, S2, BI4, FOLD>), dim3(grid), dim3(T), lds, st, a);
+	hipLaunchKernelGGL((MWF_BAND2_KERNEL<T, K, E1, E2, TB, S2, BI4, FOLD>), dim3(grid), dim3(T), lds, st, a);
 }
 
 template <int T, int K, int E1, int E2, bool BI4 = false>
@@ -907,16 +957,16 @@
 	hipError_t e;
 	if constexpr (is_span(T, K) || (T == 512 && K >= 4)) {
 		if (!seq2) return 0;
-		e = tb ? hipOccupancyMaxActiveBlocksPerMultiprocessor(&n, wfa_band2_kernel<T, K, E1, E2, true, true, BI4>, T, lds)
-		       : hipOccupancyMaxActiveBlocksPerMultiprocessor(&n, wfa_band2_kernel<T, K, E1, E2, false, true, BI4>, T, lds);
+		e = tb ? hipOccupancyMaxActiveBlocksPerMultiprocessor(&n, MWF_BAND2_KERNEL<T, K, E1, E2, true, true, BI4>, T, lds)
+		       : hipOccupancyMaxActiveBlocksPerMultiprocessor(&n, MWF_BAND2_KERNEL<T, K, E1, E2, false, true, BI4>, T, lds);
 	} else if constexpr (T == 768) {
 		if (seq2) return 0;
-		e = tb ? hipOccupancyMaxActiveBlocksPerMultiprocessor(&n, wfa_band2_kernel<T, K, E1, E2, true, false>, T, lds)
-		       : hipOccupancyMaxActiveBlocksPerMultiprocessor(&n, wfa_band2_kernel<T, K, E1, E2, false, false>, T, lds);
+		e = tb ? hipOccupancyMaxActiveBlocksPerMultiprocessor(&n, MWF_BAND2_KERNEL<T, K, E1, E2, true, false>, T, lds)
+		       : hipOccupancyMaxActiveBlocksPerMultiprocessor(&n, MWF_BAND2_KERNEL<T, K, E1, E2, false, false>, T, lds);
 	} else {
 		if (!seq2) return 0;
-		e = tb ? hipOccupancyMaxActiveBlocksPerMultiprocessor(&n, wfa_band2_kernel<T, K, E1, E2, true, true>, T, lds)
-		       : hipOccupancyMaxActiveBlocksPerMultiprocessor(&n, wfa_band2_kernel<T, K, E1, E2, false, true>, T, lds);
+		e = tb ? hipOccupancyMaxActiveBlocksPerMultiprocessor(&n, MWF_BAND2_KERNEL<T, K, E1, E2, true, true>, T, lds)
+		       : hipOccupancyMaxActiveBlocksPerMultiprocessor(&n, MWF_BAND2_KERNEL<T, K, E1, E2, false, true>, T, lds);
 	}
 	return e == hipSuccess ? n : 0;
 }
@@ -933,8 +983,11 @@
 int launch_band2_bi2(const BatchArgs &a, int grid, const BandGeom &g, void *stream);
 int band2_occupancy_bi1(const Penalty &p, const BandGeom &g, bool cigar);
 int band2_occupancy_bi2(const Penalty &p, const BandGeom &g, bool cigar);
-
-#if !defined(MWF_BAND2_DEEP) && !defined(MWF_BAND2_BIASED)
+int launch_band2_tab(const BatchArgs &a, int grid, const BandGeom &g, void *stream);
+int band2_occupancy_tab(const Penalty &p, const BandGeom &g, bool cigar);
+bool band2_tab_supported(const Penalty &p, bool band_fold);
+
+#if !defined(MWF_BAND2_DEEP) && !defined(MWF_BAND2_BIASED) && !defined(MWF_BAND2_TAB)
 bool band2_supported(const Penalty &p)
 {
 	const bool deep = (p.e1 == 3 && (p.e2 == 1 || p.e2 == 2)) || (p.e1 == 4 && p.e2 == 1);
@@ -1014,7 +1067,60 @@
 		MWF_BAND2_REST(FN, __VA_ARGS__)                                             \
 	} while (0)
 
-#if defined(MWF_BAND2_BIASED)
+#if defined(MWF_BAND2_TAB)
+namespace {
+bool tab_geom_ok(const Penalty &p, const BandGeom &g)
+{
+	return g.packed == 1 && g.block == 512 && g.seq2 != 0 && g.tab > 0 && g.tab % 16 == 0 && g.lds_bytes > g.tab && band2_tab_supported(p, true);
+}
+template <int K, bool TB>
+int launch_tab(const BatchArgs &a, int grid, int lds, hipStream_t st)
+{
+	if (lds > 48 * 1024) {
+		(void)hipFuncSetAttribute(reinterpret_cast<const void*>(&MWF_BAND2_KERNEL<512, K, 2, 1, TB, true, false, true>), hipFuncAttributeMaxDynamicSharedMemorySize, lds);
+		(void)hipGetLastError();
+	}
+	if (getenv("MWF_DEBUG")) {
+		fprintf(stderr, "[libmwf_hip] band2 launch: T %d K %d E1 %d E2 %d TB %d S2 %d BI4 %d FOLD %d, %d pairs, grid %d\n", 512, K, 2, 1, (int)TB, 1, 0, 1, (int)a.n_pairs, grid);
+		fprintf(stderr, "[libmwf_hip] band2 table probe: table %d B, lds %d B\n", (int)a.band_lds_tab, lds);
+	}
+	hipLaunchKernelGGL((MWF_BAND2_KERNEL<512, K, 2, 1, TB, true, false, true>), dim3(grid), dim3(512), lds, st, a);
+	return hipGetLastError() == hipSuccess ? 0 : -2;
+}
+template <int K, bool TB>
+int occ_tab(int lds)
+{
+	int n = 0;
+	return hipOccupancyMaxActiveBlocksPerMultiprocessor(&n, MWF_BAND2_KERNEL<512, K, 2, 1, TB, true, false, true>, 512, lds) == hipSuccess ? n : 0;
+}
+}
+
+bool band2_tab_supported(const Penalty &p, bool band_fold)
+{
+	return band_fold && p.e1 == 2 && p.e2 == 1 && p.oe1 - p.x == p.e1 && p.oe1 < kFoldMaxLag;
+}
+
+int launch_band2_tab(const BatchArgs &a0, int grid, const BandGeom &g, void *stream)
+{
+	if (!tab_geom_ok(a0.pen, g) || !a0.band_fold) return -1;
+	BatchArgs a = a0;
+	a.band_lds_seq = g.lds_bytes, a.band_lds_tab = g.tab;
+	const bool four = g.span > 512 / 64 * 3 * 256;
+	const int lds = g.lds_bytes + (four ? lds_tail<512, 4, 2, 1>() : lds_tail<512, 3, 2, 1>());
+	hipStream_t st = (hipStream_t)stream;
+	if (four) return a.want_cigar ? launch_tab<4, true>(a, grid, lds, st) : launch_tab<4, false>(a, grid, lds, st);
+	return a.want_cigar ? launch_tab<3, true>(a, grid, lds, st) : launch_tab<3, false>(a, grid, lds, st);
+}
+
+int band2_occupancy_tab(const Penalty &p, const BandGeom &g, bool cigar)
+{
+	if (!tab_geom_ok(p, g)) return 0;
+	const bool four = g.span > 512 / 64 * 3 * 256;
+	const int lds = g.lds_bytes + (four ? lds_tail<512, 4, 2, 1>() : lds_tail<512, 3, 2, 1>());
+	if (four) return cigar ? occ_tab<4, true>(lds) : occ_tab<4, false>(lds);
+	return cigar ? occ_tab<3, true>(lds) : occ_tab<3, false>(lds);
+}
+#elif defined(MWF_BAND2_BIASED)
 int MWF_BAND2_CAT(launch_band2_bi, MWF_BAND2_BIASED)(const BatchArgs &a, int grid, const BandGeom &g, void *stream)
 {
 	const int a_e1 = a.pen.e1, a_e2 = a.pen.e2;
@@ -1047,9 +1153,15 @@
 	return 0;
 }
 #else
-int launch_band2(const BatchArgs &a, int grid, const BandGeom &g, void *stream)
+int launch_band2(const BatchArgs &a, int grid, const BandGeom &g0, void *stream)
 {
 	const int a_e1 = a.pen.e1, a_e2 = a.pen.e2;
+	BandGeom g = g0;
+	if (g.tab > 0) {
+		const int rc = launch_band2_tab(a, grid, g, stream);
+		if (rc != -1) return rc;
+		g.lds_bytes -= g.tab, g.tab = 0;
+	}
 	if (g.packed == 2 && !(a_e1 == 2 && a_e2 == 1)) return a_e1 <= 2 ? launch_band2_bi1(a, grid, g, stream) : launch_band2_bi2(a, grid, g, stream);
 	if (a_e1 == 3) return launch_band2_e3(a, grid, g, stream);
 	if (a_e1 == 4) return launch_band2_e4(a, grid, g, stream);
@@ -1067,6 +1179,7 @@
 int band2_kernel_occupancy(const Penalty &p, const BandGeom &g, bool cigar)
 {
 	const int a_e1 = p.e1, a_e2 = p.e2;
+	if (g.tab > 0) return band2_occupancy_tab(p, g, cigar);
 	if (g.packed == 2 && !(a_e1 == 2 && a_e2 == 1)) return a_e1 <= 2 ? band2_occupancy_bi1(p, g, cigar) : band2_occupancy_bi2(p, g, cigar);
 	if (a_e1 == 3) return band2_occupancy_e3(p, g, cigar);
 	if (a_e1 == 4) return band2_occupancy_e4(p, g, cigar);
diff --git a/miniwfa_amd/csrc/mwf_band2_tab.hip b/miniwfa_amd/csrc/mwf_band2_tab.hip
--- /dev/null
+++ b/miniwfa_amd/csrc/mwf_band2_tab.hip
@@ -0,0 +1,2 @@
+#define MWF_BAND2_TAB 1
+#include "mwf_band2.hip"
diff --git a/miniwfa_amd/csrc/mwf_engine.cpp b/miniwfa_amd/csrc/mwf_engine.cpp
--- a/miniwfa_amd/csrc/mwf_engine.cpp
+++ b/miniwfa_amd/csrc/mwf_engine.cpp
@@ -77,6 +77,7 @@
 	else if (!strcmp(name, "div_aware")) g->div_aware = value != 0;
 	else if (!strcmp(name, "dev_retry")) g->dev_retry = value != 0;
 	else if (!strcmp(name, "band_fold")) g->band_fold = value != 0;
+	else if (!strcmp(name, "probe_table")) g->probe_table = value != 0;
 	else if (!strcmp(name, "trim")) { (void)hipSetDevice(g->device); trim(g); }
 	else return -1;
 	++g->tun_gen;
@@ -94,6 +95,7 @@
 	else if (!strcmp(name, "lane_chunks") && value >= 0 && value <= 4) g->lane_chunks = (int)value;
 	else if (!strcmp(name, "mid_block") && (value == 0 || value == 256 || value == 512 || value == 1024)) g->mid_block = (int)value;
 	else if (!strcmp(name, "lds_e2")) g->lds_e2 = value != 0;
+	else if (!strcmp(name, "probe_table_lds")) g->probe_table_lds = std::max<int64_t>(0, value);
 	else if (!strcmp(name, "scalar_generic")) g->scalar_generic = value != 0;
 	else if (!strcmp(name, "coop_spin_limit")) g->coop_spin_limit = std::max<int64_t>(0, std::min<int64_t>(value, 0x7fffffff));
 	else if (!strcmp(name, "coop_tb_cap_mb")) g->coop_tb_cap = std::max<int64_t>(1, value) << 20;
diff --git a/miniwfa_amd/csrc/mwf_engine.h b/miniwfa_amd/csrc/mwf_engine.h
--- a/miniwfa_amd/csrc/mwf_engine.h
+++ b/miniwfa_amd/csrc/mwf_engine.h
@@ -61,6 +61,8 @@
 	int retry_mode = 0;
 	int retry_slot = 0;
 	bool band_fold = true;
+	bool probe_table = true;
+	int64_t probe_table_lds = 0;
 	bool div_aware = true;
 	int64_t tun_gen = 0;
 	int64_t coop_min_len = 0;
diff --git a/miniwfa_amd/csrc/mwf_internal.h b/miniwfa_amd/csrc/mwf_internal.h
--- a/miniwfa_amd/csrc/mwf_internal.h
+++ b/miniwfa_amd/csrc/mwf_internal.h
@@ -116,6 +116,7 @@
 	int32_t lane_chunks;
 	int32_t sys_coop_launch;
 	int64_t *timeline;
+	int32_t band_lds_tab;
 };
 
 int launch_reset(int32_t *status, int32_t *s, int32_t n, unsigned long long *cig_head, int32_t *queue, int32_t n_queue, void *stream);
@@ -149,6 +150,7 @@
 	int lds_bytes;
 	int seq2;
 	int lane;
+	int tab;
 };
 bool coop_supported(const Penalty &p);
 int64_t coop_chunk_slots(int grid);
@@ -178,6 +180,7 @@
 bool band2_supported(const Penalty &p);
 int  launch_band2(const BatchArgs &a, int grid, const BandGeom &g, void *stream);
 int  band2_kernel_occupancy(const Penalty &p, const BandGeom &g, bool cigar);
+bool band2_tab_supported(const Penalty &p, bool band_fold);
 bool band2_biased512_supported(const Penalty &p);
 int  band2_biased512_chunks();
 int  band2_span_chunks();
diff --git a/miniwfa_amd/csrc/mwf_plan.cpp b/miniwfa_amd/csrc/mwf_plan.cpp
--- a/miniwfa_amd/csrc/mwf_plan.cpp
+++ b/miniwfa_amd/csrc/mwf_plan.cpp
@@ -95,7 +95,7 @@
 	}
 	const int64_t max_window = window_hint > 0 ? std::min<int64_t>(std::min<int64_t>(max_len + 1, 2 * max_bound + 3), window_hint) : std::min<int64_t>(max_len + 1, 2 * max_bound + 3);
 	BandGeom bg;
-	bg.packed = 0, bg.seq2 = 0, bg.lane = 0;
+	bg.packed = 0, bg.seq2 = 0, bg.lane = 0, bg.tab = 0;
 	const bool range_ok = max_tl + max_bound < 32767;
 	if (!range_ok) return;
 	bg.packed = 1;
@@ -103,7 +103,7 @@
 	if (g->block == 64 || g->block == 128 || g->block == 256 || g->block == 512 || g->block == 768) bg.block = g->block;
 	if (g->block == 0 && (geom_block == 64 || geom_block == 128 || geom_block == 256)) bg.block = geom_block;
 	bg.span = bg.block / 64 * (bg.block != 768 ? 3 : 2) * 256;
-	const bool four_slots = bg.block == 512 && g->block == 0 && window_hint > kBandWideWindow && window_hint <= kBandWide4Window;
+	const bool four_slots = bg.block == 512 && ((g->block == 0 && window_hint > kBandWideWindow && window_hint <= kBandWide4Window) || (g->block == 512 && g->wide_slots == 4));
 	if (four_slots) bg.span = 512 / 64 * 4 * 256;
 	if (want_kind != 2 && max_len + 1 > 4 * (int64_t)bg.span) return;
 	const int64_t lds_cap = bg.block >= 768 ? 140 * 1024 : bg.block >= 512 ? 70 * 1024 : bg.block == 256 ? 36 * 1024 : bg.block == 128 ? 18 * 1024 : 9 * 1024;
@@ -118,6 +118,15 @@
 	}
 	if (bg.lds_bytes == 0) return;
 	pl.kind = 2, pl.band = bg;
+	if (g->probe_table && bg.block == 512 && bg.seq2 && band2_tab_supported(P, g->band_fold)) {
+		const int64_t tab = (2 * (max_len + 258) + 15) / 16 * 16;
+		const int64_t budget = g->probe_table_lds > 0 ? g->probe_table_lds : (160 / 2 - 6) * 1024;
+		if (tab + bg.lds_bytes <= budget) {
+			pl.band.tab = (int)tab, pl.band.lds_bytes = (int)(tab + bg.lds_bytes);
+			pl.cigar = (opt.flag & MWF_F_CIGAR) != 0;
+			if (cached_occupancy(g, P, pl, 0, false) < 2) pl.band = bg;
+		}
+	}
 }
 
 int cached_occupancy(mwf_gpu_t *g, const Penalty &P, const Plan &pl, int lds_e2_cols, bool stream_pass, bool ring16)
@@ -125,7 +134,7 @@
 	uint64_t key;
 	if (pl.kind == 2)
 		key = 1ull | (uint64_t)pl.band.block << 4 | (uint64_t)(pl.band.packed == 1) << 16 | (uint64_t)(pl.band.packed == 2) << 15 | (uint64_t)(pl.band.lds_bytes > 0) << 17 | (uint64_t)pl.cigar << 18 |
-		      (uint64_t)(pl.band.seq2 != 0) << 3 | (uint64_t)(pl.band.lane == 1) << 2 | (uint64_t)(pl.band.block == 512 && pl.band.span > 6144) << 1 | (uint64_t)(pl.band.block == 512 ? pl.band.span / 2048 : 0) << 56 | (uint64_t)(pl.band.lane == 2) << 19 | (uint64_t)P.e1 << 20 | (uint64_t)P.e2 << 28 | (uint64_t)pl.band.lds_bytes << 36;
+		      (uint64_t)(pl.band.seq2 != 0) << 3 | (uint64_t)(pl.band.lane == 1) << 2 | (uint64_t)(pl.band.block == 512 && pl.band.span > 6144) << 1 | (uint64_t)(pl.band.block == 512 ? pl.band.span / 2048 : 0) << 56 | (uint64_t)(pl.band.lane == 2) << 19 | (uint64_t)P.e1 << 20 | (uint64_t)P.e2 << 28 | (uint64_t)pl.band.lds_bytes << 36 | (uint64_t)(pl.band.tab > 0) << 62;
 	else key = 2ull | (uint64_t)pl.block << 4 | (uint64_t)stream_pass << 16 | (uint64_t)ring16 << 17 | (uint64_t)(P.nH > kMaxRing) << 18 | (uint64_t)lds_e2_cols << 20;
 	auto it = g->occ_cache.find(key);
 	if (it != g->occ_cache.end()) return it->second;
diff --git a/profiles/timing_probe_band2_chunk.py b/profiles/timing_probe_band2_chunk.py
--- a/profiles/timing_probe_band2_chunk.py
+++ b/profiles/timing_probe_band2_chunk.py
@@ -7,6 +7,7 @@
 from miniwfa_amd.synth import synth_pair, PackedBatch
 eng = mw.Engine(0)
 if len(sys.argv) > 1: eng.set("band_fold", int(sys.argv[1]))
+if len(sys.argv) > 2: eng.set("probe_table", int(sys.argv[2]))
 for n in (1, 512):
     b = eng.upload(PackedBatch([synth_pair(50000, 10000, 0.05)] * n))
     o = mw.opt_init()
```

New measurement: 1.663 Gbp/s (median of 6 runs). +7.9%, better.
